# SysCV/LiDAR_snow_sim

Hardware: NVIDIA H100
Metric: augmented LiDAR points/sec (higher is better)
Workload: dtype f64

## Files before the change

### lidar_snow_sim_b200/csrc/api.cu

```cuda
#include "common.cuh"
#include <cmath>
#include <cstring>
#include <cstdlib>

namespace {

void host_range_grid(double *R)
{
    const double stop = 120 + 299792458.0 * 1e-8;
    const double step = stop / (LSS_M_EXT - 1);
    for (int k = 0; k < LSS_M_EXT; k++) {
        double v = (k == LSS_M_EXT - 1) ? stop : k * step;
        R[k] = std::nearbyint(v * 100.0) / 100.0;
    }
}

void host_phase_table(const double *R, double *tab )
{
    const long double ctau = (long double)(299792458.0 * 1e-8);
    const long double pi = 3.14159265358979323846264338327950288L;
    for (int k = 0; k < LSS_M_EXT; k++) {
        const long double a = fmodl((long double)R[k] / ctau, 2.0L);
        tab[2 * k] = (double)sinl(pi * a);
        tab[2 * k + 1] = (double)cosl(pi * a);
    }
}

}

extern "C" {

int lss_version(void) { return 100; }

const char *lss_status_string(lss_status s)
{
    switch (s) {
        case LSS_OK: return "ok";
        case LSS_ERR_INVALID_ARG: return "invalid argument";
        case LSS_ERR_CUDA: return "CUDA error";
        case LSS_ERR_NO_TABLE: return "particle table set not found";
        case LSS_ERR_RANGE_INDEX: return "waveform index out of range (return beyond ~120 m on an occluded beam)";
        case LSS_ERR_NEGATIVE_INTENSITY: return "new intensity is negative";
        case LSS_ERR_OCCLUDER_OVERFLOW: return "too many occluders on one beam";
        case LSS_ERR_WORKSPACE: return "workspace too small";
        case LSS_ERR_NO_SENSOR: return "sensor / camera constants not set";
        case LSS_ERR_TOO_FEW_GROUND: return "fewer than 3 ground points: laser parameters cannot be estimated";
        case LSS_ERR_INTENSITY_RANGE:
            return "intensity histogram range (5, max(I/cos)) of the ground points is not finite or max is below 5";
    }
    return "unknown status";
}

const char *lss_last_error(const lss_engine *e) { return e ? e->last_error.c_str() : "null engine"; }

lss_status lss_create(int device, lss_engine **out)
{
    if (!out) return LSS_ERR_INVALID_ARG;
    *out = nullptr;
    int n_dev = 0;
    if (cudaGetDeviceCount(&n_dev) != cudaSuccess || n_dev == 0) return LSS_ERR_CUDA;
    if (device < 0 || device >= n_dev) return LSS_ERR_INVALID_ARG;
    lss_engine *e = new lss_engine();
    e->device = device;
    DeviceGuard g(device);
    double R[LSS_M_EXT];
    host_range_grid(R);
    std::vector<double> wtab(2 * LSS_M_EXT);
    host_phase_table(R, wtab.data());
    int zero = 0;
    cudaDeviceGetAttribute(&e->n_sm, cudaDevAttrMultiProcessorCount, device);
    if (e->n_sm <= 0) e->n_sm = 132;
    if (cudaMalloc(&e->d_R, sizeof(R)) != cudaSuccess || cudaMalloc(&e->d_status, sizeof(int)) != cudaSuccess ||
        cudaMalloc(&e->d_wtab, sizeof(double) * wtab.size()) != cudaSuccess ||
        cudaMemcpy(e->d_wtab, wtab.data(), sizeof(double) * wtab.size(), cudaMemcpyHostToDevice) != cudaSuccess ||
        cudaMalloc(&e->d_sensor, sizeof(SensorConst)) != cudaSuccess ||
        cudaMalloc(&e->d_camera, sizeof(CameraConst)) != cudaSuccess ||
        cudaMemcpy(e->d_R, R, sizeof(R), cudaMemcpyHostToDevice) != cudaSuccess ||
        cudaMemcpy(e->d_status, &zero, sizeof(int), cudaMemcpyHostToDevice) != cudaSuccess) {
        lss_destroy(e);
        return LSS_ERR_CUDA;
    }
    *out = e;
    return LSS_OK;
}

void lss_destroy(lss_engine *e)
{
    if (!e) return;
    DeviceGuard g(e->device);
    for (auto &kv : e->tables) {
        cudaFree(kv.second.d_rec);
        cudaFree(kv.second.d_tan);
        cudaFree(kv.second.d_plane_off);
        cudaFree(kv.second.d_entries);
        cudaFree(kv.second.d_bucket_start);
    }
    cudaFree(e->d_R);
    cudaFree(e->d_wtab);
    cudaFree(e->d_status);
    cudaFree(e->d_sensor);
    cudaFree(e->d_camera);
    lss_host_pipe_free(e);
    for (cudaStream_t st : e->side) if (st) { cudaStreamSynchronize(st); cudaStreamDestroy(st); }
    for (cudaEvent_t ev : e->side_ev) if (ev) cudaEventDestroy(ev);
    for (auto &sl : e->stage) {
        if (sl.done) { cudaEventSynchronize(sl.done); cudaEventDestroy(sl.done); }
        if (sl.host) cudaFreeHost(sl.host);
    }
    delete e;
}

lss_status lss_set_sensor(lss_engine *e, int n_channels, const double *fd, const double *fs, const double *mi,
                          const double *mx)
{
    if (!e || !fd || !fs || !mi || !mx) return LSS_ERR_INVALID_ARG;
    if (n_channels != LSS_N_CHANNELS) return lss_fail(e, LSS_ERR_INVALID_ARG, "n_channels must be 64");
    DeviceGuard g(e->device);
    for (int c = 0; c < LSS_N_CHANNELS; c++) {
        const double focal_distance = fd[c] * 100;
        const double t = 1 - focal_distance / 13100;
        e->sensor.focal_offset[c] = t * t;
        e->sensor.focal_slope[c] = fs[c];
        e->sensor.min_intensity[c] = mi[c];
        e->sensor.max_intensity[c] = mx[c];
    }
    LSS_CUDA_CHECK(e, cudaMemcpy(e->d_sensor, &e->sensor, sizeof(SensorConst), cudaMemcpyHostToDevice));
    e->has_sensor = true;
    return LSS_OK;
}

lss_status lss_set_camera(lss_engine *e, const float *P2, const float *R0, const float *V2C, int img_h, int img_w)
{
    if (!e || !P2 || !R0 || !V2C) return LSS_ERR_INVALID_ARG;
    DeviceGuard g(e->device);
    for (int k = 0; k < 4; k++)
        for (int j = 0; j < 3; j++) {
            float acc = 0.0f;
            for (int m = 0; m < 3; m++) acc = fmaf(V2C[m * 4 + k], R0[j * 3 + m], acc);
            e->camera.M[k * 3 + j] = acc;
        }
    memcpy(e->camera.P2, P2, sizeof(float) * 12);
    e->camera.img_h = img_h;
    e->camera.img_w = img_w;
    LSS_CUDA_CHECK(e, cudaMemcpy(e->d_camera, &e->camera, sizeof(CameraConst), cudaMemcpyHostToDevice));
    e->has_camera = true;
    return LSS_OK;
}

static lss_status upload_common(lss_engine *e, int n_planes, const double *d_xyr, const int64_t *h_off, double max_div,
                                int n_buckets, cudaStream_t stream, int *id_out)
{
    if (n_planes <= 0 || !h_off || !id_out) return lss_fail(e, LSS_ERR_INVALID_ARG, "bad table arguments");
    if (n_buckets <= 0) n_buckets = 2048;
    if (n_buckets < 8 || n_buckets > (1 << 16)) return lss_fail(e, LSS_ERR_INVALID_ARG, "n_azimuth_buckets out of range");
    if (!(max_div > 0) || max_div > 1.0) return lss_fail(e, LSS_ERR_INVALID_ARG, "max_beam_divergence_rad out of range");
    for (int k = 0; k < n_planes; k++)
        if (h_off[k + 1] < h_off[k] || h_off[0] != 0) return lss_fail(e, LSS_ERR_INVALID_ARG, "bad plane offsets");
    TableSet ts;
    ts.n_planes = n_planes;
    ts.n_buckets = n_buckets;
    ts.max_div_rad = max_div;
    lss_status st = lss_build_tables(e, ts, d_xyr, h_off, stream);
    if (st != LSS_OK) {
        cudaFree(ts.d_rec);
        cudaFree(ts.d_tan);
        cudaFree(ts.d_plane_off);
        cudaFree(ts.d_entries);
        cudaFree(ts.d_bucket_start);
        return st;
    }
    const int id = e->next_table_id++;
    e->tables[id] = ts;
    *id_out = id;
    return LSS_OK;
}

lss_status lss_upload_particles(lss_engine *e, int n_planes, const double *h_xyr, const int64_t *h_off, double max_div,
                                int n_buckets, void *stream, int *id_out)
{
    if (!e || !h_xyr || !h_off) return LSS_ERR_INVALID_ARG;
    DeviceGuard g(e->device);
    cudaStream_t st = (cudaStream_t)stream;
    const int64_t np = n_planes > 0 ? h_off[n_planes] : 0;
    if (np <= 0) return lss_fail(e, LSS_ERR_INVALID_ARG, "empty particle table set");
    double *d_xyr = nullptr;
    LSS_CUDA_CHECK(e, cudaMalloc(&d_xyr, sizeof(double) * 3 * np));
    cudaError_t ce = cudaMemcpyAsync(d_xyr, h_xyr, sizeof(double) * 3 * np, cudaMemcpyHostToDevice, st);
    lss_status r = LSS_OK;
    if (ce != cudaSuccess) {
        e->last_error = cudaGetErrorString(ce);
        r = LSS_ERR_CUDA;
    } else {
        r = upload_common(e, n_planes, d_xyr, h_off, max_div, n_buckets, st, id_out);
    }
    cudaStreamSynchronize(st);
    cudaFree(d_xyr);
    return r;
}

lss_status lss_upload_particles_device(lss_engine *e, int n_planes, const double *d_xyr, const int64_t *h_off,
                                       double max_div, int n_buckets, void *stream, int *id_out)
{
    if (!e || !d_xyr || !h_off) return LSS_ERR_INVALID_ARG;
    DeviceGuard g(e->device);
    return upload_common(e, n_planes, d_xyr, h_off, max_div, n_buckets, (cudaStream_t)stream, id_out);
}

lss_status lss_free_particles(lss_engine *e, int table_id)
{
    if (!e) return LSS_ERR_INVALID_ARG;
    auto it = e->tables.find(table_id);
    if (it == e->tables.end()) return lss_fail(e, LSS_ERR_NO_TABLE, "unknown table id");
    DeviceGuard g(e->device);
    cudaFree(it->second.d_rec);
    cudaFree(it->second.d_tan);
    cudaFree(it->second.d_plane_off);
    cudaFree(it->second.d_entries);
    cudaFree(it->second.d_bucket_start);
    e->tables.erase(it);
    return LSS_OK;
}

lss_status lss_table_info(lss_engine *e, int table_id, int64_t *n_particles, int64_t *n_entries, int64_t *bytes)
{
    if (!e) return LSS_ERR_INVALID_ARG;
    auto it = e->tables.find(table_id);
    if (it == e->tables.end()) return lss_fail(e, LSS_ERR_NO_TABLE, "unknown table id");
    if (n_particles) *n_particles = it->second.n_particles;
    if (n_entries) *n_entries = it->second.n_entries;
    if (bytes) *bytes = it->second.bytes;
    return LSS_OK;
}

int64_t lss_snowfall_workspace_bytes(int64_t n_total, int n_clouds) { return lss_snowfall_ws_bytes(n_total, n_clouds); }

lss_status lss_snowfall_batch(lss_engine *e, int table_id, const float *d_points, const int64_t *h_cloud_offsets,
                              int n_clouds, const int32_t *h_order, double beam_divergence_deg, const float *d_theta,
                              const double *h_thresh_poly, const double *h_plane_in, const int32_t *h_ymins_in,
                              double noise_floor, uint32_t flags, float *d_out_points,
                              int32_t *d_out_counts, double *d_out_stats, float *d_out_full, int32_t *d_out_perm,
                              int32_t *d_out_nocc, void *d_workspace, int64_t workspace_bytes, void *stream)
{
    return lss_snowfall_batch_slots(e, table_id, d_points, h_cloud_offsets, nullptr, n_clouds, h_order,
                                    beam_divergence_deg, d_theta, h_thresh_poly, h_plane_in, h_ymins_in, noise_floor,
                                    flags, d_out_points, d_out_counts, d_out_stats, d_out_full, d_out_perm, d_out_nocc,
                                    d_workspace, workspace_bytes, stream);
}

lss_status lss_snowfall_batch_slots(lss_engine *e, int table_id, const float *d_points, const int64_t *h_cloud_offsets,
                                    const int32_t *d_cloud_counts, int n_clouds, const int32_t *h_order,
                                    double beam_divergence_deg, const float *d_theta, const double *h_thresh_poly,
                                    const double *h_plane_in, const int32_t *h_ymins_in, double noise_floor,
                                    uint32_t flags, float *d_out_points, int32_t *d_out_counts, double *d_out_stats,
                                    float *d_out_full, int32_t *d_out_perm, int32_t *d_out_nocc, void *d_workspace,
                                    int64_t workspace_bytes, void *stream)
{
    if (!e) return LSS_ERR_INVALID_ARG;
    if (!h_cloud_offsets || !h_order || n_clouds < 0 || !d_out_points || !d_out_counts || !d_out_stats)
        return lss_fail(e, LSS_ERR_INVALID_ARG, "null argument");
    if (!d_points && n_clouds <= 65535 && h_cloud_offsets[n_clouds] > 0) return lss_fail(e, LSS_ERR_INVALID_ARG, "null points");
    if (!e->has_sensor) return lss_fail(e, LSS_ERR_NO_SENSOR, "sensor constants not set (lss_set_sensor)");
    auto it = e->tables.find(table_id);
    if (it == e->tables.end()) return lss_fail(e, LSS_ERR_NO_TABLE, "unknown table id");
    DeviceGuard g(e->device);
    SnowfallArgs a;
    a.ts = &it->second;
    a.d_points = d_points;
    a.h_cloud_offsets = h_cloud_offsets;
    a.d_cloud_counts = d_cloud_counts;
    a.n_clouds = n_clouds;
    a.h_order = h_order;
    a.beam_divergence_deg = beam_divergence_deg;
    a.d_theta = d_theta;
    a.h_thresh_poly = h_thresh_poly;
    a.h_plane_in = h_plane_in;
    a.h_ymins_in = h_ymins_in;
    a.noise_floor = noise_floor;
    a.flags = flags;
    a.d_out_points = d_out_points;
    a.d_out_counts = d_out_counts;
    a.d_out_stats = d_out_stats;
    a.d_out_full = d_out_full;
    a.d_out_perm = d_out_perm;
    a.d_out_nocc = d_out_nocc;
    a.d_workspace = d_workspace;
    a.workspace_bytes = workspace_bytes;
    return lss_snowfall_run(e, a, (cudaStream_t)stream);
}

static int64_t *poly_carve(WsCarve &c, void *&pre, int64_t &pre_bytes, int64_t n_total, int n_clouds)
{
    int64_t *off = c.take<int64_t>(n_clouds + 1);
    pre_bytes = lss_prepass_ws_bytes(n_total, n_clouds);
    pre = c.take<char>(pre_bytes);
    return off;
}

int64_t lss_prepass_workspace_bytes(int64_t n_total, int n_clouds)
{
    if (n_total < 0 || n_clouds < 0) return -1;
    WsCarve c;
    void *pre;
    int64_t pre_bytes;
    poly_carve(c, pre, pre_bytes, n_total, n_clouds);
    return c.used;
}

lss_status lss_noise_threshold_poly(lss_engine *e, const float *d_points, const int64_t *h_cloud_offsets, int n_clouds,
                                    double noise_floor, const double *h_plane_in, const int32_t *h_ymins_in,
                                    double *d_poly_out, double *d_plane_out, double *d_fit_out, int32_t *d_ymins_out,
                                    void *d_workspace, int64_t workspace_bytes, void *stream)
{
    if (!e) return LSS_ERR_INVALID_ARG;
    if (!d_points || n_clouds <= 0 || !d_poly_out || !d_workspace) return lss_fail(e, LSS_ERR_INVALID_ARG, "null argument");
    BatchGeometry geo;
    if (lss_status rc = lss_batch_geometry(e, h_cloud_offsets, n_clouds, 0, geo)) return rc;
    DeviceGuard g(e->device);
    if (lss_status rc = lss_prepass_check(e, h_cloud_offsets, n_clouds, h_plane_in != nullptr)) return rc;
    cudaStream_t st = (cudaStream_t)stream;
    WsCarve c{(char *)d_workspace};
    void *d_pre;
    int64_t pre_bytes;
    int64_t *d_off = poly_carve(c, d_pre, pre_bytes, geo.n, n_clouds);
    if (workspace_bytes < c.used) return lss_fail(e, LSS_ERR_WORKSPACE, "workspace too small");
    LSS_CUDA_CHECK(e, lss_stage_upload(e, d_off, h_cloud_offsets, sizeof(int64_t) * (n_clouds + 1), st));
    PrepassIO io;
    io.h_plane_in = h_plane_in;
    io.h_ymins_in = h_ymins_in;
    io.d_poly_out = d_poly_out;
    io.d_plane_out = d_plane_out;
    io.d_fit_out = d_fit_out;
    io.d_ymins_out = d_ymins_out;
    return lss_prepass_run(e, d_points, d_off, nullptr, h_cloud_offsets, n_clouds, 0.5, noise_floor, 0, 0, 1, io,
                           d_pre, pre_bytes, nullptr, st);
}

lss_status lss_check_async(lss_engine *e, void *stream)
{
    if (!e) return LSS_ERR_INVALID_ARG;
    DeviceGuard g(e->device);
    cudaStream_t st = (cudaStream_t)stream;
    int code = 0, zero = 0;
    LSS_CUDA_CHECK(e, cudaStreamSynchronize(st));
    LSS_CUDA_CHECK(e, cudaMemcpyAsync(&code, e->d_status, sizeof(int), cudaMemcpyDeviceToHost, st));
    LSS_CUDA_CHECK(e, cudaStreamSynchronize(st));
    if (code != 0) {
        LSS_CUDA_CHECK(e, cudaMemcpyAsync(e->d_status, &zero, sizeof(int), cudaMemcpyHostToDevice, st));
        LSS_CUDA_CHECK(e, cudaStreamSynchronize(st));
        e->last_error = lss_status_string((lss_status)code);
    }
    return (lss_status)code;
}

int64_t lss_launch_count(const lss_engine *e) { return e ? e->launches : 0; }

lss_status lss_set_profiling(lss_engine *e, int enable)
{
    if (!e) return LSS_ERR_INVALID_ARG;
    e->profiling = enable != 0;
    return LSS_OK;
}

static const char *kernel_names[LSS_K_COUNT] = {"channel_sort", "prepass", "snowfall", "compact", "keep", "wet_ground", "fog",
                                                "snowfall_scan", "snowfall_solve", "voxelize", "dror", "lisa", "fog_lut", "mie",
                                                "select", "pa_aug"};

const char *lss_kernel_name(int kernel) { return (kernel >= 0 && kernel < LSS_K_COUNT) ? kernel_names[kernel] : ""; }

lss_status lss_kernel_times(lss_engine *e, int reset, double *h_ms, int64_t *h_calls, int n)
{
    if (!e || !h_ms || !h_calls) return LSS_ERR_INVALID_ARG;
    DeviceGuard g(e->device);
    for (auto &t : e->timed) {
        float ms = 0.0f;
        if (cudaEventSynchronize(t.end) == cudaSuccess && cudaEventElapsedTime(&ms, t.beg, t.end) == cudaSuccess) {
            e->kernel_ms[t.kernel] += ms;
            e->kernel_calls[t.kernel]++;
        }
        cudaEventDestroy(t.beg);
        cudaEventDestroy(t.end);
    }
    e->timed.clear();
    for (int k = 0; k < n && k < LSS_K_COUNT; k++) { h_ms[k] = e->kernel_ms[k]; h_calls[k] = e->kernel_calls[k]; }
    if (reset) for (int k = 0; k < 16; k++) { e->kernel_ms[k] = 0; e->kernel_calls[k] = 0; }
    return LSS_OK;
}

lss_status lss_debug_range_grid(double *h_out)
{
    if (!h_out) return LSS_ERR_INVALID_ARG;
    host_range_grid(h_out);
    return LSS_OK;
}

}
```

### lidar_snow_sim_b200/csrc/common.cuh

```cuda
#pragma once
#include <cuda_runtime.h>
#include <stdint.h>
#include <stdio.h>
#include <string>
#include <vector>
#include <cstring>
#include <map>
#include <utility>

#include "../../include/lidar_snow_sim.h"

#define LSS_PI 3.141592653589793
#define LSS_TWO_PI 6.283185307179586
#define LSS_M_EXT 1230
#define LSS_ANG_MARGIN 1e-5

struct ParticleRec {
    double phi;
    double rho;
    double alpha;
};
struct ParticleTan {
    double t_right, t_left;
};

typedef uint2 BroadEntry;
#define LSS_RHO_UNIT 0.0025f
#define LSS_RHO_PER_M 400.0
#define LSS_PHI_UNIT 9.587672516830327e-05
#define LSS_IDX_BITS 22
struct EntryView { float x, y, z; int idx; };
__device__ __forceinline__ EntryView lss_decode(const BroadEntry raw, float zbase)
{
    EntryView v;
    v.x = (float)(raw.x & 0xffffu) * LSS_RHO_UNIT;
    v.y = (float)((int)raw.x >> 16) * (float)LSS_PHI_UNIT;
    v.z = zbase * exp2f((float)(raw.y >> LSS_IDX_BITS) * (1.0f / 32.0f));
    v.idx = (int)(raw.y & ((1u << LSS_IDX_BITS) - 1u));
    return v;
}

struct TableSet {
    int n_planes = 0;
    int n_buckets = 0;
    double max_div_rad = 0.0;
    int64_t n_particles = 0;
    int64_t n_entries = 0;
    float zbase = 0.0f;
    ParticleRec *d_rec = nullptr;
    ParticleTan *d_tan = nullptr;
    BroadEntry *d_entries = nullptr;
    int32_t *d_bucket_start = nullptr;
    int64_t *d_plane_off = nullptr;
    int64_t bytes = 0;
};

struct SensorConst {
    double focal_offset[LSS_N_CHANNELS];
    double focal_slope[LSS_N_CHANNELS];
    double min_intensity[LSS_N_CHANNELS];
    double max_intensity[LSS_N_CHANNELS];
};

struct CameraConst {
    float M[12];
    float P2[12];
    int img_h, img_w;
};

__device__ __forceinline__ bool lss_camera_fov(const CameraConst *cam, float out_x, float out_y, float out_z,
                                               const int *img_h, const int *img_w)
{
    const float *M = cam->M, *P2 = cam->P2;
    float rx = fmaf(out_z, M[6], fmaf(out_y, M[3], out_x * M[0])) + M[9];
    float ry = fmaf(out_z, M[7], fmaf(out_y, M[4], out_x * M[1])) + M[10];
    float rz = fmaf(out_z, M[8], fmaf(out_y, M[5], out_x * M[2])) + M[11];
    float u = fmaf(rz, P2[2], fmaf(ry, P2[1], rx * P2[0])) + P2[3];
    float v = fmaf(rz, P2[6], fmaf(ry, P2[5], rx * P2[4])) + P2[7];
    float wd = fmaf(rz, P2[10], fmaf(ry, P2[9], rx * P2[8])) + P2[11];
    u = u / rz;
    v = v / rz;
    const float depth = wd - P2[11];
    return (u >= 0.0f) && (u < (float)*img_w) && (v >= 0.0f) && (v < (float)*img_h) && (depth >= 0.0f);
}

struct lss_host_pipe;
struct lss_engine {
    int device = 0;
    bool has_sensor = false;
    bool has_camera = false;
    SensorConst sensor;
    CameraConst camera;
    SensorConst *d_sensor = nullptr;
    CameraConst *d_camera = nullptr;
    double *d_R = nullptr;
    double2 *d_wtab = nullptr;
    int n_sm = 132;
    int *d_status = nullptr;
    std::map<int, TableSet> tables;
    int next_table_id = 1;
    int64_t launches = 0;
    std::string last_error;
    bool profiling = false;
    struct TimedLaunch { int kernel; cudaEvent_t beg, end; };
    std::vector<TimedLaunch> timed;
    double kernel_ms[16] = {0};
    int64_t kernel_calls[16] = {0};
    struct StageSlot { void *host = nullptr; size_t cap = 0; cudaEvent_t done = nullptr; };
    static constexpr int N_STAGE = 256;
    StageSlot stage[N_STAGE];
    int stage_next = 0;
    static constexpr int N_SIDE = 4;
    cudaStream_t side[N_SIDE] = {};
    cudaEvent_t side_ev[2 * 32] = {};
    int side_next = 0;
    struct lss_host_pipe *pipe = nullptr;
};
void lss_host_pipe_free(lss_engine *e);

inline int64_t align_up(int64_t v, int64_t al) { return (v + al - 1) / al * al; }

struct WsCarve {
    char *base = nullptr;
    int64_t used = 0;
    template <typename T> T *take(int64_t count)
    {
        T *p = base ? (T *)(base + used) : nullptr;
        used = align_up(used + count * (int64_t)sizeof(T), 256);
        return p;
    }
};

template <typename... P, typename... A>
[[nodiscard]] inline cudaError_t lss_launch(lss_engine *e, void (*kernel)(P...), dim3 grid, dim3 block, size_t smem,
                                            cudaStream_t stream, A &&...args)
{
    kernel<<<grid, block, smem, stream>>>(std::forward<A>(args)...);
    e->launches++;
    return cudaGetLastError();
}

inline cudaError_t lss_side_stream(lss_engine *e, cudaStream_t *stream, cudaEvent_t *ev_fork, cudaEvent_t *ev_join)
{
    cudaError_t err;
    const int k = e->side_next++;
    cudaStream_t &s = e->side[k % lss_engine::N_SIDE];
    if (!s) {
        int least = 0, greatest = 0;
        if ((err = cudaDeviceGetStreamPriorityRange(&least, &greatest)) != cudaSuccess) return err;
        if ((err = cudaStreamCreateWithPriority(&s, cudaStreamNonBlocking, greatest)) != cudaSuccess) return err;
    }
    cudaEvent_t *ev = &e->side_ev[2 * (k % 32)];
    for (int j = 0; j < 2; j++)
        if (!ev[j] && (err = cudaEventCreateWithFlags(&ev[j], cudaEventDisableTiming)) != cudaSuccess) return err;
    *stream = s; *ev_fork = ev[0]; *ev_join = ev[1];
    return cudaSuccess;
}

static __global__ void k_stage_copy(uint32_t *dst, const uint32_t *src, int n_words)
{
    for (int i = blockIdx.x * blockDim.x + threadIdx.x; i < n_words; i += gridDim.x * blockDim.x) dst[i] = src[i];
}

inline cudaError_t lss_stage_upload(lss_engine *e, void *dst, const void *src, size_t bytes, cudaStream_t stream)
{
    if (bytes == 0) return cudaSuccess;
    if (bytes % 4 != 0 || ((uintptr_t)dst & 3) != 0) return cudaErrorInvalidValue;
    lss_engine::StageSlot &sl = e->stage[e->stage_next];
    e->stage_next = (e->stage_next + 1) % lss_engine::N_STAGE;
    cudaError_t err;
    if (!sl.done) {
        if ((err = cudaEventCreateWithFlags(&sl.done, cudaEventDisableTiming)) != cudaSuccess) return err;
    } else if ((err = cudaEventSynchronize(sl.done)) != cudaSuccess) {
        return err;
    }
    if (sl.cap < bytes) {
        if (sl.host) cudaFreeHost(sl.host);
        sl.host = nullptr; sl.cap = 0;
        const size_t cap = bytes < 4096 ? 4096 : bytes * 2;
        if ((err = cudaHostAlloc(&sl.host, cap, cudaHostAllocMapped)) != cudaSuccess) return err;
        sl.cap = cap;
    }
    memcpy(sl.host, src, bytes);
    const int n_words = (int)(bytes / 4);
    const int blocks = n_words >= 1 << 16 ? 64 : (n_words + 1023) / 1024;
    if ((err = lss_launch(e, k_stage_copy, blocks, 256, 0, stream, (uint32_t *)dst, (const uint32_t *)sl.host, n_words)) !=
        cudaSuccess)
        return err;
    return cudaEventRecord(sl.done, stream);
}

struct ZeroRegions {
    static constexpr int MAX = 6;
    uint32_t *p[MAX];
    unsigned long long words[MAX];
    int n = 0;
    void add(void *ptr, size_t bytes) { if (ptr && bytes) { p[n] = (uint32_t *)ptr; words[n] = (bytes + 3) / 4; n++; } }
};
static __global__ void k_zero_regions(ZeroRegions r)
{
    uint32_t *p = r.p[blockIdx.y];
    const unsigned long long n = r.words[blockIdx.y];
    const unsigned long long stride = (unsigned long long)gridDim.x * blockDim.x;
    for (unsigned long long i = (unsigned long long)blockIdx.x * blockDim.x + threadIdx.x; i < n; i += stride) p[i] = 0u;
}
inline cudaError_t lss_zero_async(lss_engine *e, const ZeroRegions &r, cudaStream_t stream)
{
    if (r.n == 0) return cudaSuccess;
    unsigned long long mx = 0;
    for (int i = 0; i < r.n; i++) mx = r.words[i] > mx ? r.words[i] : mx;
    const unsigned long long cap = 4ull * e->n_sm;
    const unsigned blocks = (unsigned)((mx + 1023) / 1024 < cap ? (mx + 1023) / 1024 : cap);
    return lss_launch(e, k_zero_regions, dim3(blocks ? blocks : 1, r.n), 256, 0, stream, r);
}

enum { LSS_K_SORT = 0, LSS_K_PREPASS = 1, LSS_K_SNOWFALL = 2, LSS_K_COMPACT = 3, LSS_K_FINALIZE = 4, LSS_K_WET = 5,
       LSS_K_FOG = 6, LSS_K_SCAN = 7, LSS_K_SOLVE = 8, LSS_K_VOXEL = 9, LSS_K_DROR = 10, LSS_K_LISA = 11,
       LSS_K_FOG_LUT = 12, LSS_K_MIE = 13, LSS_K_SELECT = 14, LSS_K_PA = 15, LSS_K_COUNT = 16 };

struct KernelTimer {
    lss_engine *e; cudaStream_t s; int idx = -1;
    KernelTimer(lss_engine *e_, int kernel, cudaStream_t s_) : e(e_), s(s_) {
        if (!e->profiling) return;
        lss_engine::TimedLaunch t; t.kernel = kernel;
        cudaEventCreate(&t.beg); cudaEventCreate(&t.end);
        cudaEventRecord(t.beg, s);
        e->timed.push_back(t); idx = (int)e->timed.size() - 1;
    }
    ~KernelTimer() { if (idx >= 0) cudaEventRecord(e->timed[idx].end, s); }
};

#define LSS_CUDA_CHECK(e, call)                                                                          \
    do {                                                                                                 \
        cudaError_t _err = (call);                                                                       \
        if (_err != cudaSuccess) {                                                                       \
            char _buf[512];                                                                              \
            snprintf(_buf, sizeof(_buf), "%s failed: %s (%s:%d)", #call, cudaGetErrorString(_err),      \
                     __FILE__, __LINE__);                                                                \
            (e)->last_error = _buf;                                                                      \
            return LSS_ERR_CUDA;                                                                         \
        }                                                                                                \
    } while (0)

struct DeviceGuard {
    int prev = -1;
    explicit DeviceGuard(int dev) { cudaGetDevice(&prev); if (prev != dev) cudaSetDevice(dev); else prev = -1; }
    ~DeviceGuard() { if (prev >= 0) cudaSetDevice(prev); }
};

static inline lss_status lss_fail(lss_engine *e, lss_status s, const char *msg)
{
    if (e) e->last_error = msg;
    return s;
}

struct BatchGeometry {
    int64_t n = 0, max_n = 0;
    std::vector<int32_t> tile_base;
};

inline lss_status lss_batch_geometry(lss_engine *e, const int64_t *h_cloud_offsets, int n_clouds, int tile,
                                     BatchGeometry &g)
{
    if (!h_cloud_offsets || n_clouds < 0) return lss_fail(e, LSS_ERR_INVALID_ARG, "null argument");
    if (n_clouds > 65535) return lss_fail(e, LSS_ERR_INVALID_ARG, "at most 65535 clouds per call");
    if (h_cloud_offsets[0] != 0) return lss_fail(e, LSS_ERR_INVALID_ARG, "cloud_offsets[0] must be 0");
    g.max_n = 0;
    g.tile_base.assign(tile > 0 ? n_clouds + 1 : 0, 0);
    for (int b = 0; b < n_clouds; b++) {
        const int64_t n = h_cloud_offsets[b + 1] - h_cloud_offsets[b];
        if (n < 0) return lss_fail(e, LSS_ERR_INVALID_ARG, "cloud_offsets must be non-decreasing");
        if (n >= (1LL << 31)) return lss_fail(e, LSS_ERR_INVALID_ARG, "cloud too large");
        g.max_n = n > g.max_n ? n : g.max_n;
        if (tile > 0) g.tile_base[b + 1] = g.tile_base[b] + (int32_t)((n + tile - 1) / tile);
    }
    g.n = h_cloud_offsets[n_clouds];
    return LSS_OK;
}

inline cudaError_t lss_stage_geometry(lss_engine *e, const int64_t *h_cloud_offsets, int n_clouds,
                                      const std::vector<int32_t> &tile_base, int64_t *d_off, int32_t *d_tile_base,
                                      cudaStream_t stream)
{
    const cudaError_t err = lss_stage_upload(e, d_off, h_cloud_offsets, sizeof(int64_t) * (n_clouds + 1), stream);
    if (err != cudaSuccess) return err;
    return lss_stage_upload(e, d_tile_base, tile_base.data(), sizeof(int32_t) * tile_base.size(), stream);
}

lss_status lss_build_tables(lss_engine *e, TableSet &ts, const double *d_xyr, const int64_t *h_plane_offsets,
                            cudaStream_t stream);
struct SnowfallArgs {
    const TableSet *ts;
    const float *d_points;
    const int64_t *h_cloud_offsets;
    const int32_t *d_cloud_counts = nullptr;
    int n_clouds;
    const int32_t *h_order;
    double beam_divergence_deg;
    const float *d_theta;
    const double *h_thresh_poly;
    const double *h_plane_in = nullptr;
    const int32_t *h_ymins_in = nullptr;
    double noise_floor;
    uint32_t flags;
    float *d_out_points;
    int32_t *d_out_counts;
    double *d_out_stats;
    float *d_out_full;
    int32_t *d_out_perm;
    int32_t *d_out_nocc;
    void *d_workspace;
    int64_t workspace_bytes;
};
lss_status lss_snowfall_run(lss_engine *e, const SnowfallArgs &a, cudaStream_t stream);
struct CloudPre {
    double w[3], h;
    double nw;
    int n_window;
    int n_ground;
    double ymax;
    double lin[2];
    double pmin[2];
    double poly[3];
    float z_med, mad;
    int best_trial;
    int flat;
    double mom[11];
};
__device__ __forceinline__ bool lss_intensity_range_ok(double ymax) { return ymax >= 5.0 && !isinf(ymax); }
__device__ __forceinline__ double lss_plane_dot(double x, double y, double z, const double *w)
{
    return __dadd_rn(__dadd_rn(__dmul_rn(x, w[0]), __dmul_rn(y, w[1])), __dmul_rn(z, w[2]));
}
int64_t lss_prepass_ws_bytes(int64_t n_total, int n_clouds);
struct PrepassIO {
    const double *h_plane_in = nullptr;
    const int32_t *h_ymins_in = nullptr;
    double *d_poly_out = nullptr;
    double *d_plane_out = nullptr;
    double *d_fit_out = nullptr;
    int32_t *d_ymins_out = nullptr;
    int range_min_ground = 3;
};
lss_status lss_prepass_run(lss_engine *e, const float *d_pts, const int64_t *d_cloud_off, const int32_t *d_cloud_cnt,
                           const int64_t *h_cloud_off, int n_clouds, double delta, double noise_floor, int flat_earth,
                           int range64, int raise_few_ground, const PrepassIO &io, void *d_ws, int64_t ws_bytes,
                           void **cloudpre_out, cudaStream_t stream);
lss_status lss_prepass_check(lss_engine *e, const int64_t *h_cloud_off, int n_clouds, bool plane_given);
int64_t lss_snowfall_ws_bytes(int64_t n_total, int n_clouds);
struct DevArgs;
int *lss_snowfall_carve(WsCarve &c, DevArgs &a, void *&prepass, int64_t n_total, int n_clouds);
```

### lidar_snow_sim_b200/csrc/prepass.cu

```cuda
#include "common.cuh"

namespace {

constexpr int PP_TPB = 256;
constexpr int HIST_NX = 50, HIST_NY = 2555;
constexpr int RANSAC_T = 128;


struct PreArgs {
    const float *pts;
    const int64_t *cloud_off;
    const int32_t *cloud_cnt;
    int raise_few;
    int range_min_ground;
    int range64;
    int n_clouds;
    double delta;
    double noise_floor;
    int flat_earth;
    int have_plane;
    CloudPre *cp;
    float *win;
    float *stage;
    int *tile_cnt;
    const int32_t *tile_base;
    double *rec_norm;
    unsigned char *rec_bin;
    int *rec_cnt;
    double *trial;
    double *partial;
    int max_blocks;
    int *status;
    const int32_t *ymins_in;
    int32_t *ymins;
};

__device__ __forceinline__ float range32(float x, float y, float z)
{
    return __fsqrt_rn(__fadd_rn(__fadd_rn(__fmul_rn(x, x), __fmul_rn(y, y)), __fmul_rn(z, z)));
}

__device__ __forceinline__ unsigned long long splitmix64(unsigned long long x)
{
    x += 0x9E3779B97F4A7C15ULL;
    x = (x ^ (x >> 30)) * 0xBF58476D1CE4E5B9ULL;
    x = (x ^ (x >> 27)) * 0x94D049BB133111EBULL;
    return x ^ (x >> 31);
}

template <int NV>
__device__ void block_sum(double (&v)[NV], double *smem )
{
    const int lane = threadIdx.x & 31, warp = threadIdx.x >> 5, nw = blockDim.x >> 5;
#pragma unroll
    for (int k = 0; k < NV; k++)
#pragma unroll
        for (int s = 16; s > 0; s >>= 1) v[k] += __shfl_down_sync(0xffffffffu, v[k], s);
    __syncthreads();
    if (lane == 0)
#pragma unroll
        for (int k = 0; k < NV; k++) smem[k * nw + warp] = v[k];
    __syncthreads();
    if (threadIdx.x == 0)
#pragma unroll
        for (int k = 0; k < NV; k++) {
            double s = 0.0;
            for (int q = 0; q < nw; q++) s += smem[k * nw + q];
            v[k] = s;
        }
}

constexpr int WTILE = 256;

__device__ __forceinline__ bool lss_in_window(float x, float y, float z)
{
    const float lim = __fsub_rn(-1.86f, __fmul_rn(0.01f, x));
    return (z < -1.55f) && (z > lim) && (x > 10.0f) && (x < 70.0f) && (y > -3.0f) && (y < 3.0f);
}
__device__ __forceinline__ int64_t lss_window_tile0(int64_t cloud_begin, int b) { return cloud_begin / 32 + b; }

__global__ void __launch_bounds__(WTILE) k_window_tiles(PreArgs a)
{
    const int b = blockIdx.y;
    const int64_t beg = a.cloud_off[b];
    const int n = (a.cloud_cnt ? a.cloud_cnt[b] : (int)(a.cloud_off[b + 1] - beg));
    const int w0 = blockIdx.x * WTILE + (threadIdx.x & ~31);
    if (w0 >= n) return;
    const int lane = threadIdx.x & 31;
    const int i = w0 + lane;
    float x = 0, y = 0, z = 0;
    bool in = false;
    if (i < n) {
        const float *r = a.pts + (beg + i) * 5;
        x = __ldcs(r); y = __ldcs(r + 1); z = __ldcs(r + 2);
        in = lss_in_window(x, y, z);
    }
    const unsigned m = __ballot_sync(0xffffffffu, in);
    if (in) {
        float *o = a.stage + (beg + w0 + __popc(m & ((1u << lane) - 1u))) * 3;
        o[0] = x; o[1] = y; o[2] = z;
    }
    if (lane == 0) a.tile_cnt[lss_window_tile0(beg, b) + w0 / 32] = __popc(m);
}

__device__ __forceinline__ unsigned f2key(float f)
{
    unsigned u = __float_as_uint(f);
    return (u & 0x80000000u) ? ~u : (u | 0x80000000u);
}
__device__ __forceinline__ float key2f(unsigned k)
{
    unsigned u = (k & 0x80000000u) ? (k & 0x7fffffffu) : ~k;
    return __uint_as_float(u);
}

__device__ float block_select(const float *win, int K, int kth, int mode, float centre, unsigned *hist ,
                              unsigned *bcast )
{
    unsigned prefix = 0, mask = 0;
    int k = kth;
    for (int shift = 24; shift >= 0; shift -= 8) {
        for (int q = threadIdx.x; q < 256; q += blockDim.x) hist[q] = 0;
        __syncthreads();
        for (int i = threadIdx.x; i < K; i += blockDim.x) {
            float v = win[3 * (size_t)i + 2];
            if (mode) v = fabsf(__fsub_rn(v, centre));
            const unsigned key = f2key(v);
            if ((key & mask) == prefix) atomicAdd(&hist[(key >> shift) & 255u], 1u);
        }
        __syncthreads();
        if (threadIdx.x == 0) {
            int acc = 0;
            unsigned d = 0;
            for (; d < 256; d++) {
                if (acc + (int)hist[d] > k) break;
                acc += (int)hist[d];
            }
            bcast[0] = d;
            bcast[1] = (unsigned)(k - acc);
        }
        __syncthreads();
        prefix |= bcast[0] << shift;
        mask |= 255u << shift;
        k = (int)bcast[1];
        __syncthreads();
    }
    return key2f(prefix);
}

__device__ float block_median(const float *win, int K, int mode, float centre, unsigned *hist, unsigned *bcast)
{
    const float hi = block_select(win, K, K / 2, mode, centre, hist, bcast);
    if (K & 1) return hi;
    const float lo = block_select(win, K, K / 2 - 1, mode, centre, hist, bcast);
    return __fmul_rn(__fadd_rn(lo, hi), 0.5f);
}

__global__ void __launch_bounds__(1024) k_window_gather_mad(PreArgs a)
{
    extern __shared__ int prefix[];
    __shared__ int wsum[32];
    __shared__ int run_s;
    __shared__ unsigned hist[256];
    __shared__ unsigned bcast[2];
    const int b = blockIdx.x;
    const int64_t beg = a.cloud_off[b];
    const int n = (a.cloud_cnt ? a.cloud_cnt[b] : (int)(a.cloud_off[b + 1] - beg));
    const int n_tiles = (n + 31) / 32;
    const int *cnt = a.tile_cnt + lss_window_tile0(beg, b);
    const int tid = threadIdx.x, lane = tid & 31, warp = tid >> 5;
    if (tid == 0) run_s = 0;
    __syncthreads();
    for (int base = 0; base < n_tiles; base += 1024) {
        const int t = base + tid;
        const int v = t < n_tiles ? cnt[t] : 0;
        int incl = v;
#pragma unroll
        for (int s = 1; s < 32; s <<= 1) { const int o = __shfl_up_sync(0xffffffffu, incl, s); if (lane >= s) incl += o; }
        if (lane == 31) wsum[warp] = incl;
        __syncthreads();
        int o = run_s;
        for (int wv = 0; wv < warp; wv++) o += wsum[wv];
        if (t < n_tiles) prefix[t] = o + incl - v;
        __syncthreads();
        if (tid == 1023) run_s = o + incl;
        __syncthreads();
    }
    if (tid == 0) { prefix[n_tiles] = run_s; a.cp[b].n_window = run_s; }
    __syncthreads();
    const int K = prefix[n_tiles];
    float *win = a.win + beg * 3;
    for (int o = tid; o < K; o += blockDim.x) {
        int lo = 0, hi = n_tiles;
        while (hi - lo > 1) { const int mid = (lo + hi) >> 1; if (prefix[mid] <= o) lo = mid; else hi = mid; }
        const float *src = a.stage + (beg + (int64_t)lo * 32 + (o - prefix[lo])) * 3;
        float *dst = win + (int64_t)o * 3;
        dst[0] = src[0]; dst[1] = src[1]; dst[2] = src[2];
    }
    if (K <= 5) return;
    __syncthreads();
    const float med = block_median(win, K, 0, 0.0f, hist, bcast);
    const float mad = block_median(win, K, 1, med, hist, bcast);
    if (threadIdx.x == 0) { a.cp[b].z_med = med; a.cp[b].mad = mad; }
}

__global__ void __launch_bounds__(PP_TPB) k_ransac_trials(PreArgs a)
{
    __shared__ double red[5 * (PP_TPB / 32)];
    __shared__ double model[4];
    const int b = blockIdx.y, t = blockIdx.x;
    const int K = a.cp[b].n_window;
    double *out = a.trial + ((size_t)b * RANSAC_T + t) * 8;
    if (K <= 5) { if (threadIdx.x == 0) out[5] = 0.0; return; }
    const float *win = a.win + a.cloud_off[b] * 3;
    if (threadIdx.x == 0) {
        unsigned long long s = splitmix64(0x5851F42D4C957F2DULL ^ ((unsigned long long)(unsigned)K << 32) ^ (unsigned)t);
        int i0 = (int)(s % (unsigned)K);
        s = splitmix64(s);
        int i1 = (int)(s % (unsigned)(K - 1));
        if (i1 >= i0) i1++;
        s = splitmix64(s);
        int i2 = (int)(s % (unsigned)(K - 2));
        const int lo = i0 < i1 ? i0 : i1, hi = i0 < i1 ? i1 : i0;
        if (i2 >= lo) i2++;
        if (i2 >= hi) i2++;
        const double x0 = win[3 * i0], y0 = win[3 * i0 + 1], z0 = win[3 * i0 + 2];
        const double x1 = win[3 * i1] - x0, y1 = win[3 * i1 + 1] - y0, z1 = win[3 * i1 + 2] - z0;
        const double x2 = win[3 * i2] - x0, y2 = win[3 * i2 + 1] - y0, z2 = win[3 * i2 + 2] - z0;
        const double det = x1 * y2 - x2 * y1;
        double valid = 0.0, pa = 0, pb = 0, pc = 0;
        if (fabs(det) > 1e-9) {
            pa = (z1 * y2 - z2 * y1) / det;
            pb = (x1 * z2 - x2 * z1) / det;
            pc = z0 - pa * x0 - pb * y0;
            valid = 1.0;
        }
        model[0] = pa; model[1] = pb; model[2] = pc; model[3] = valid;
    }
    __syncthreads();
    if (model[3] == 0.0) { if (threadIdx.x == 0) out[5] = 0.0; return; }
    const double pa = model[0], pb = model[1], pc = model[2];
    const double thr = (double)a.cp[b].mad;
    double v[5] = {0, 0, 0, 0, 0};
    for (int i = threadIdx.x; i < K; i += PP_TPB) {
        const double x = win[3 * i], y = win[3 * i + 1], z = win[3 * i + 2];
        const double r = z - (pa * x + pb * y + pc);
        const double r2 = r * r;
        if (r2 <= thr) { v[0] += 1.0; v[1] += r2; v[2] += z; v[3] += z * z; }
    }
    block_sum<5>(v, red);
    if (threadIdx.x == 0) {
        const double n = v[0];
        const double ss_tot = v[3] - (n > 0 ? v[2] * v[2] / n : 0.0);
        out[0] = n;
        out[1] = (n > 0 && ss_tot > 0) ? 1.0 - v[1] / ss_tot : -1e300;
        out[2] = pa; out[3] = pb; out[4] = pc;
        out[5] = n >= 3 ? 1.0 : 0.0;
    }
}

__global__ void __launch_bounds__(PP_TPB) k_ransac_refit(PreArgs a)
{
    __shared__ double red[6 * (PP_TPB / 32)];
    __shared__ double bc[8];
    const int b = blockIdx.x;
    CloudPre &cp = a.cp[b];
    const int K = cp.n_window;
    if (threadIdx.x < 32) {
        int best = -1;
        double bn = -1, bs = -1e301;
        for (int t = threadIdx.x; t < RANSAC_T && K > 5; t += 32) {
            const double *tr = a.trial + ((size_t)b * RANSAC_T + t) * 8;
            if (tr[5] == 0.0) continue;
            if (tr[0] > bn || (tr[0] == bn && tr[1] > bs)) { bn = tr[0]; bs = tr[1]; best = t; }
        }
#pragma unroll
        for (int sft = 16; sft > 0; sft >>= 1) {
            const double on = __shfl_xor_sync(0xffffffffu, bn, sft), os = __shfl_xor_sync(0xffffffffu, bs, sft);
            const int ob = __shfl_xor_sync(0xffffffffu, best, sft);
            const bool take = ob >= 0 && (best < 0 || on > bn || (on == bn && (os > bs || (os == bs && ob < best))));
            if (take) { bn = on; bs = os; best = ob; }
        }
        if (threadIdx.x == 0) {
        cp.best_trial = best;
        bc[0] = (double)best;
        if (best >= 0) {
            const double *tr = a.trial + ((size_t)b * RANSAC_T + best) * 8;
            bc[1] = tr[2]; bc[2] = tr[3]; bc[3] = tr[4];
        }
        }
    }
    __syncthreads();
    const int best = (int)bc[0];
    if (best < 0) {
        if (threadIdx.x == 0) { cp.w[0] = 0; cp.w[1] = 0; cp.w[2] = 1; cp.h = -1.55; cp.nw = 1.0; cp.flat = 1; }
        return;
    }
    const float *win = a.win + a.cloud_off[b] * 3;
    const double pa = bc[1], pb = bc[2], pc = bc[3], thr = (double)cp.mad;
    double m[6] = {0, 0, 0, 0, 0, 0};
    for (int i = threadIdx.x; i < K; i += PP_TPB) {
        const double x = win[3 * i], y = win[3 * i + 1], z = win[3 * i + 2];
        const double r = z - (pa * x + pb * y + pc);
        if (r * r <= thr) { m[0] += 1.0; m[1] += x; m[2] += y; m[3] += z; }
    }
    block_sum<6>(m, red);
    if (threadIdx.x == 0) { bc[4] = m[0]; bc[5] = m[1] / m[0]; bc[6] = m[2] / m[0]; bc[7] = m[3] / m[0]; }
    __syncthreads();
    const double xm = bc[5], ym = bc[6], zm = bc[7];
    double c[6] = {0, 0, 0, 0, 0, 0};
    for (int i = threadIdx.x; i < K; i += PP_TPB) {
        const double x = win[3 * i], y = win[3 * i + 1], z = win[3 * i + 2];
        const double r = z - (pa * x + pb * y + pc);
        if (r * r <= thr) {
            const double dx = x - xm, dy = y - ym, dz = z - zm;
            c[0] += dx * dx; c[1] += dx * dy; c[2] += dy * dy; c[3] += dx * dz; c[4] += dy * dz;
        }
    }
    block_sum<6>(c, red);
    if (threadIdx.x == 0) {
        const double det = c[0] * c[2] - c[1] * c[1];
        double fa = pa, fb = pb, fc = pc;
        if (fabs(det) > 1e-12 * (c[0] * c[2] + 1e-300)) {
            fa = (c[3] * c[2] - c[4] * c[1]) / det;
            fb = (c[0] * c[4] - c[1] * c[3]) / det;
            fc = zm - fa * xm - fb * ym;
        }
        const double nrm = sqrt(fa * fa + fb * fb + 1.0);
        cp.w[0] = fa / nrm; cp.w[1] = fb / nrm; cp.w[2] = -1.0 / nrm; cp.h = fc;
        cp.nw = sqrt(cp.w[0] * cp.w[0] + cp.w[1] * cp.w[1] + cp.w[2] * cp.w[2]);
        cp.flat = 0;
    }
}

__global__ void k_set_plane(PreArgs a, const double *plane )
{
    const int b = blockIdx.x * blockDim.x + threadIdx.x;
    if (b >= a.n_clouds) return;
    CloudPre &cp = a.cp[b];
    cp.w[0] = plane[4 * b]; cp.w[1] = plane[4 * b + 1]; cp.w[2] = plane[4 * b + 2]; cp.h = plane[4 * b + 3];
    cp.nw = sqrt(cp.w[0] * cp.w[0] + cp.w[1] * cp.w[1] + cp.w[2] * cp.w[2]);
    cp.flat = 0;
    cp.best_trial = -2;
}

struct GroundPt { bool ground; double d, cosang, norm_i; };

__device__ __forceinline__ GroundPt ground_point(const PreArgs &a, const CloudPre &cp, const float *r)
{
    GroundPt g;
    const double x = r[0], y = r[1], z = r[2];
    const double pw = lss_plane_dot(x, y, z, cp.w);
    const double hgt = pw + cp.h;
    g.ground = (hgt < a.delta) && (hgt > -a.delta);
    if (!g.ground) { g.d = 0.0; g.cosang = 0.0; g.norm_i = 0.0; return g; }
    g.d = a.range64 ? sqrt((x * x + y * y) + z * z) : (double)range32(r[0], r[1], r[2]);
    double c;
    if (a.flat_earth) c = -(z) / (g.d * 1.0);
    else c = pw / (g.d * cp.nw);
    g.cosang = (c >= -1.0 && c <= 1.0) ? c : __longlong_as_double(0x7ff8000000000000LL);
    g.norm_i = (double)r[3] / g.cosang;
    return g;
}

__device__ __forceinline__ int edge_bin(double v, double lo, double hi, int nb)
{
    if (!(v >= lo) || !(v <= hi)) return -1;
    const double step = (hi - lo) / nb;
    int k = (int)((v - lo) / step);
    k = k < 0 ? 0 : (k > nb ? nb : k);
    while (k > 0 && v < ((k == nb) ? hi : (k * step + lo))) k--;
    while (k < nb && v >= ((k + 1 == nb) ? hi : ((k + 1) * step + lo))) k++;
    if (k >= nb) k = nb - 1;
    return k;
}

__device__ __forceinline__ void intensity_edges(double ymax, double &lo, double &hi)
{
    lo = ymax == 5.0 ? 4.5 : 5.0;
    hi = ymax == 5.0 ? 5.5 : ymax;
}

__device__ __forceinline__ double nan_max(double a, double b) { return (a != a || a > b) ? a : b; }

__device__ __forceinline__ int ground_blocks(int n, int launched)
{
    return min(launched, max(1, (n + PP_TPB * 8 - 1) / (PP_TPB * 8)));
}

__global__ void __launch_bounds__(PP_TPB) k_ground_stats(PreArgs a)
{
    __shared__ double red[15 * (PP_TPB / 32)];
    __shared__ double mx[PP_TPB / 32];
    const int b = blockIdx.y;
    const CloudPre cp = a.cp[b];
    const int64_t beg = a.cloud_off[b];
    const int n = (a.cloud_cnt ? a.cloud_cnt[b] : (int)(a.cloud_off[b + 1] - beg));
    const int nb = ground_blocks(n, gridDim.x);
    if ((int)blockIdx.x >= nb) return;
    const int lane = threadIdx.x & 31;
    double v[15] = {0, 0, 0, 0, 0, 0, 0, 0, 0, 0, 0, 0, 0, 0, 0};
    double vmax = -1e300;
    for (int w0 = blockIdx.x * PP_TPB + (threadIdx.x & ~31); w0 < n; w0 += nb * PP_TPB) {
        const int i = w0 + lane;
        GroundPt g;
        g.ground = false;
        if (i < n) {
            const float *r = a.pts + (beg + i) * 5;
            const float row[4] = {__ldcs(r), __ldcs(r + 1), __ldcs(r + 2), __ldcs(r + 3)};
            g = ground_point(a, cp, row);
        }
        int bx = -1;
        if (g.ground) {
            const double dd = g.d - 30.0, yy = g.norm_i - 50.0;
            v[0] += 1.0; v[1] += dd; v[2] += yy; v[3] += dd * dd; v[4] += dd * yy;
            vmax = nan_max(vmax, g.norm_i);
            const double t = (g.d - 40.0) / 30.0, t2 = t * t;
            const double c = g.cosang, dc = g.d * g.cosang;
            v[5] += t; v[6] += t2; v[7] += t2 * t; v[8] += t2 * t2;
            v[9] += c; v[10] += c * t; v[11] += c * t2;
            v[12] += dc; v[13] += dc * t; v[14] += dc * t2;
            if (g.norm_i >= 4.5) bx = edge_bin(g.d, 10.0, 70.0, HIST_NX);
        }
        const unsigned m = __ballot_sync(0xffffffffu, bx >= 0);
        if (m) {
            int k0 = 0;
            if (lane == 0) k0 = atomicAdd(&a.rec_cnt[b], __popc(m));
            k0 = __shfl_sync(0xffffffffu, k0, 0);
            if (bx >= 0) {
                const int64_t k = beg + k0 + __popc(m & ((1u << lane) - 1u));
                a.rec_norm[k] = g.norm_i;
                a.rec_bin[k] = (unsigned char)bx;
            }
        }
    }
#pragma unroll
    for (int s = 16; s > 0; s >>= 1) vmax = nan_max(vmax, __shfl_down_sync(0xffffffffu, vmax, s));
    if ((threadIdx.x & 31) == 0) mx[threadIdx.x >> 5] = vmax;
    block_sum<15>(v, red);
    if (threadIdx.x == 0) {
        for (int q = 0; q < PP_TPB / 32; q++) vmax = nan_max(vmax, mx[q]);
        double *p = a.partial + ((size_t)b * a.max_blocks + blockIdx.x) * 16;
        for (int k = 0; k < 15; k++) p[k] = v[k];
        p[15] = vmax;
    }
}

template <int NV>
__device__ __forceinline__ void warp_reduce_partials(const double *partial, int n_blocks, double (&v)[NV], double *vmax)
{
    const int lane = threadIdx.x & 31;
#pragma unroll
    for (int k = 0; k < NV; k++) v[k] = 0.0;
    double m = -1e300;
    for (int q = lane; q < n_blocks; q += 32) {
        const double *p = partial + (size_t)q * 16;
#pragma unroll
        for (int k = 0; k < NV; k++) v[k] += p[k];
        if (vmax) m = nan_max(m, p[NV]);
    }
#pragma unroll
    for (int s = 16; s > 0; s >>= 1) {
#pragma unroll
        for (int k = 0; k < NV; k++) v[k] += __shfl_xor_sync(0xffffffffu, v[k], s);
        m = nan_max(m, __shfl_xor_sync(0xffffffffu, m, s));
    }
    if (vmax) *vmax = m;
}

#ifndef LSS_HIST_SLAB
#define LSS_HIST_SLAB 5
#endif
constexpr int HIST_SLAB = LSS_HIST_SLAB, HIST_SLABS = (HIST_NX + HIST_SLAB - 1) / HIST_SLAB, HIST_TPB = 512;

__global__ void __launch_bounds__(HIST_TPB) k_ground_hist(PreArgs a, int n_blocks)
{
    extern __shared__ unsigned hist[];
    __shared__ double stat[2];
    const int b = blockIdx.y, bx0 = blockIdx.x * HIST_SLAB;
    const int nbx = min(HIST_SLAB, HIST_NX - bx0);
    const int lane = threadIdx.x & 31, warp = threadIdx.x >> 5;
    if (warp == 0) {
        double v[15], vmax;
        const int n = a.cloud_cnt ? a.cloud_cnt[b] : (int)(a.cloud_off[b + 1] - a.cloud_off[b]);
        warp_reduce_partials<15>(a.partial + (size_t)b * a.max_blocks * 16, ground_blocks(n, n_blocks), v, &vmax);
        if (lane == 0) {
            stat[0] = v[0];
            stat[1] = fabs(vmax);
            if (blockIdx.x == 0) {
                CloudPre &cp = a.cp[b];
                cp.n_ground = (int)v[0];
                cp.mom[0] = v[0];
                for (int k = 0; k < 10; k++) cp.mom[1 + k] = v[5 + k];
                cp.ymax = fabs(vmax);
                if (v[0] >= 3.0) {
                    const double n = v[0], mx_ = v[1] / n, my_ = v[2] / n;
                    const double sxx = v[3] - n * mx_ * mx_, sxy = v[4] - n * mx_ * my_;
                    const double slope = sxy / sxx;
                    cp.lin[0] = slope;
                    cp.lin[1] = (my_ + 50.0) - slope * (mx_ + 30.0);
                } else {
                    cp.lin[0] = cp.lin[1] = 0.0;
                    if (a.raise_few) atomicMax(a.status, LSS_ERR_TOO_FEW_GROUND);
                }
                if (v[0] >= (double)a.range_min_ground && !lss_intensity_range_ok(cp.ymax))
                    atomicMax(a.status, LSS_ERR_INTENSITY_RANGE);
            }
        }
    }
    __syncthreads();
    const int n_ground = (int)stat[0];
    const double ymax = stat[1];
    if (n_ground < 3 || !lss_intensity_range_ok(ymax)) return;
    double ylo, yhi;
    intensity_edges(ymax, ylo, yhi);
    int32_t *ymins = a.ymins + b * HIST_NX + bx0;
    if (a.ymins_in) {
        for (int k = threadIdx.x; k < nbx; k += HIST_TPB) {
            const int inj = a.ymins_in[b * HIST_NX + bx0 + k];
            ymins[k] = inj < 0 ? 0 : (inj >= HIST_NY ? HIST_NY - 1 : inj);
        }
        return;
    }
    for (int k = threadIdx.x; k < nbx * HIST_NY; k += HIST_TPB) hist[k] = 0;
    __syncthreads();
    const int64_t beg = a.cloud_off[b];
    const int n_rec = a.rec_cnt[b];
    const unsigned char *bins = a.rec_bin + beg;
    const double *norms = a.rec_norm + beg;
    constexpr int U = 4;
    for (int k0 = threadIdx.x; k0 < n_rec; k0 += U * HIST_TPB) {
        int rel[U];
#pragma unroll
        for (int u = 0; u < U; u++) {
            const int k = k0 + u * HIST_TPB;
            rel[u] = k < n_rec ? (int)bins[k] - bx0 : -1;
        }
#pragma unroll
        for (int u = 0; u < U; u++)
            if ((unsigned)rel[u] < (unsigned)nbx) {
                const int by = edge_bin(norms[k0 + u * HIST_TPB], ylo, yhi, HIST_NY);
                if (by >= 0) atomicAdd(&hist[rel[u] * HIST_NY + by], 1u);
            }
    }
    __syncthreads();
    for (int w = warp; w < nbx; w += HIST_TPB / 32) {
        unsigned best = 0xffffffffu;
        int bidx = 0x7fffffff;
        for (int k = lane; k < HIST_NY; k += 32) {
            unsigned c = hist[w * HIST_NY + k];
            if (c == 0) c = (unsigned)n_ground;
            if (c < best) { best = c; bidx = k; }
        }
        for (int s = 16; s > 0; s >>= 1) {
            const unsigned ob = __shfl_down_sync(0xffffffffu, best, s);
            const int oi = __shfl_down_sync(0xffffffffu, bidx, s);
            if (ob < best || (ob == best && oi < bidx)) { best = ob; bidx = oi; }
        }
        if (lane == 0) ymins[w] = bidx;
    }
}

__device__ __forceinline__ bool minima_point(int k, int bidx, double ylo, double yhi, double ystep, double &x, double &y)
{
    y = (bidx == HIST_NY) ? yhi : __dadd_rn(__dmul_rn((double)bidx, ystep), ylo);
    const double e0 = k * (60.0 / HIST_NX) + 10.0;
    const double e1 = (k + 1 == HIST_NX) ? 70.0 : ((k + 1) * (60.0 / HIST_NX) + 10.0);
    x = (e0 + e1) / 2;
    return y > 5.0;
}

__global__ void k_poly_solve(PreArgs a, double *poly_out , double *plane_out ,
                             double *fit_out , int32_t *ymins_out )
{
    const int b = blockIdx.x;
    CloudPre &cp = a.cp[b];
    if (threadIdx.x != 0) return;
    const bool picked = cp.n_ground >= 3 && lss_intensity_range_ok(cp.ymax);
    if (cp.n_ground >= 3) {
        const int32_t *ymins = a.ymins + b * HIST_NX;
        double ylo, yhi;
        intensity_edges(cp.ymax, ylo, yhi);
        const double ystep = (yhi - ylo) / HIST_NY;
        int m = 0;
        double sx = 0, sy = 0, x, y;
        for (int k = 0; k < HIST_NX && picked; k++)
            if (minima_point(k, ymins[k], ylo, yhi, ystep, x, y)) { m++; sx += x; sy += y; }
        if (m > 3) {
            const double mx_ = sx / m, my_ = sy / m;
            double sxx = 0, sxy = 0;
            for (int k = 0; k < HIST_NX; k++)
                if (minima_point(k, ymins[k], ylo, yhi, ystep, x, y)) { sxx += (x - mx_) * (x - mx_); sxy += (x - mx_) * (y - my_); }
            cp.pmin[0] = sxy / sxx;
            cp.pmin[1] = my_ - cp.pmin[0] * mx_;
        } else {
            cp.pmin[0] = cp.lin[0];
            cp.pmin[1] = cp.lin[1];
        }
    }
    double s[8];
    s[0] = cp.mom[0]; s[1] = cp.mom[1]; s[2] = cp.mom[2]; s[3] = cp.mom[3]; s[4] = cp.mom[4];
    for (int k = 0; k < 3; k++) s[5 + k] = a.noise_floor * (cp.pmin[0] * cp.mom[8 + k] + cp.pmin[1] * cp.mom[5 + k]);
    double A[3][4] = {{s[0], s[1], s[2], s[5]}, {s[1], s[2], s[3], s[6]}, {s[2], s[3], s[4], s[7]}};
    bool ok = cp.n_ground >= 3;
    for (int c = 0; c < 3 && ok; c++) {
        int piv = c;
        for (int r = c + 1; r < 3; r++) if (fabs(A[r][c]) > fabs(A[piv][c])) piv = r;
        if (fabs(A[piv][c]) < 1e-300) { ok = false; break; }
        for (int k = 0; k < 4; k++) { double t = A[c][k]; A[c][k] = A[piv][k]; A[piv][k] = t; }
        for (int r = c + 1; r < 3; r++) {
            const double f = A[r][c] / A[c][c];
            for (int k = c; k < 4; k++) A[r][k] -= f * A[c][k];
        }
    }
    double c2 = 0, c1 = 0, c0 = 0;
    if (ok) {
        c2 = A[2][3] / A[2][2];
        c1 = (A[1][3] - A[1][2] * c2) / A[1][1];
        c0 = (A[0][3] - A[0][1] * c1 - A[0][2] * c2) / A[0][0];
    }
    const double m = 40.0, sc = 30.0;
    cp.poly[0] = c2 / (sc * sc);
    cp.poly[1] = c1 / sc - 2.0 * c2 * m / (sc * sc);
    cp.poly[2] = c0 - c1 * m / sc + c2 * m * m / (sc * sc);
    if (poly_out) { poly_out[3 * b] = cp.poly[0]; poly_out[3 * b + 1] = cp.poly[1]; poly_out[3 * b + 2] = cp.poly[2]; }
    if (plane_out) { plane_out[4 * b] = cp.w[0]; plane_out[4 * b + 1] = cp.w[1]; plane_out[4 * b + 2] = cp.w[2]; plane_out[4 * b + 3] = cp.h; }
    if (fit_out) {
        double *f = fit_out + 8 * b;
        f[0] = cp.lin[0]; f[1] = cp.lin[1]; f[2] = cp.pmin[0]; f[3] = cp.pmin[1]; f[4] = cp.ymax;
        f[5] = (double)cp.n_ground; f[6] = (double)cp.n_window; f[7] = (double)cp.flat;
    }
    if (ymins_out) for (int k = 0; k < HIST_NX; k++) ymins_out[b * HIST_NX + k] = picked ? a.ymins[b * HIST_NX + k] : -1;
}

}

static void prepass_carve(WsCarve &c, PreArgs &a, double *&plane_in, int32_t *&ymins_in, int64_t n_total, int n_clouds)
{
    a.max_blocks = 64;
    a.cp = c.take<CloudPre>(n_clouds);
    a.rec_cnt = c.take<int>(n_clouds);
    a.win = c.take<float>(n_total * 3);
    a.stage = c.take<float>(n_total * 3);
    a.rec_norm = (double *)a.stage;
    a.rec_bin = a.stage ? (unsigned char *)a.stage + n_total * 8 : nullptr;
    a.tile_cnt = c.take<int>(n_total / 32 + n_clouds + 2);
    a.tile_base = c.take<int32_t>(n_clouds + 1);
    a.trial = c.take<double>((int64_t)n_clouds * RANSAC_T * 8);
    a.partial = c.take<double>((int64_t)n_clouds * a.max_blocks * 16);
    plane_in = c.take<double>((int64_t)n_clouds * 4);
    a.ymins = c.take<int32_t>((int64_t)n_clouds * HIST_NX);
    ymins_in = c.take<int32_t>((int64_t)n_clouds * HIST_NX);
}

int64_t lss_prepass_ws_bytes(int64_t n_total, int n_clouds)
{
    WsCarve c;
    PreArgs a;
    double *plane_in;
    int32_t *ymins_in;
    prepass_carve(c, a, plane_in, ymins_in, n_total, n_clouds);
    return c.used;
}

static size_t gather_dyn_smem(int64_t max_n) { return sizeof(int) * ((size_t)(max_n + 31) / 32 + 2); }

static int64_t largest_cloud(const int64_t *h_cloud_off, int n_clouds)
{
    int64_t max_n = 0;
    for (int b = 0; b < n_clouds; b++) max_n = std::max<int64_t>(max_n, h_cloud_off[b + 1] - h_cloud_off[b]);
    return max_n;
}

static lss_status gather_smem_limits(lss_engine *e, size_t &static_bytes, size_t &optin_bytes)
{
    cudaFuncAttributes fa;
    int optin = 0;
    LSS_CUDA_CHECK(e, cudaFuncGetAttributes(&fa, k_window_gather_mad));
    LSS_CUDA_CHECK(e, cudaDeviceGetAttribute(&optin, cudaDevAttrMaxSharedMemoryPerBlockOptin, e->device));
    static_bytes = fa.sharedSizeBytes;
    optin_bytes = (size_t)optin;
    return LSS_OK;
}

lss_status lss_prepass_check(lss_engine *e, const int64_t *h_cloud_off, int n_clouds, bool plane_given)
{
    if (plane_given || n_clouds <= 0) return LSS_OK;
    const int64_t max_n = largest_cloud(h_cloud_off, n_clouds);
    size_t static_bytes = 0, optin_bytes = 0;
    if (lss_status rc = gather_smem_limits(e, static_bytes, optin_bytes)) return rc;
    if (static_bytes + gather_dyn_smem(max_n) <= optin_bytes) return LSS_OK;
    const int64_t limit = ((int64_t)((optin_bytes - static_bytes) / sizeof(int)) - 2) * 32;
    char msg[256];
    snprintf(msg, sizeof(msg), "pre-pass: a cloud of %lld rows is larger than the %lld rows whose mounting window this "
             "device can gather (shared memory); give its plane or split it", (long long)max_n, (long long)limit);
    e->last_error = msg;
    return LSS_ERR_INVALID_ARG;
}

lss_status lss_prepass_run(lss_engine *e, const float *d_pts, const int64_t *d_cloud_off, const int32_t *d_cloud_cnt,
                           const int64_t *h_cloud_off, int n_clouds, double delta, double noise_floor, int flat_earth,
                           int range64, int raise_few_ground, const PrepassIO &io, void *d_ws, int64_t ws_bytes,
                           void **cloudpre_out, cudaStream_t stream)
{
    const double *h_plane_in = io.h_plane_in;
    double *d_poly_out = io.d_poly_out, *d_plane_out = io.d_plane_out;
    const int B = n_clouds;
    const int64_t N = h_cloud_off[B];
    PreArgs a;
    WsCarve c{(char *)d_ws};
    double *d_plane;
    int32_t *d_ymins_in;
    prepass_carve(c, a, d_plane, d_ymins_in, N, B);
    if (lss_status rc = lss_prepass_check(e, h_cloud_off, B, h_plane_in != nullptr)) return rc;
    if (ws_bytes < c.used) return lss_fail(e, LSS_ERR_WORKSPACE, "pre-pass workspace too small");
    a.pts = d_pts;
    a.cloud_off = d_cloud_off;
    a.cloud_cnt = d_cloud_cnt;
    a.range64 = range64;
    a.raise_few = raise_few_ground;
    a.range_min_ground = io.range_min_ground;
    a.n_clouds = B;
    a.delta = delta;
    a.noise_floor = noise_floor;
    a.flat_earth = flat_earth;
    a.have_plane = h_plane_in != nullptr;
    a.status = e->d_status;
    a.ymins_in = nullptr;
    if (io.h_ymins_in) {
        LSS_CUDA_CHECK(e, lss_stage_upload(e, d_ymins_in, io.h_ymins_in, sizeof(int32_t) * HIST_NX * B, stream));
        a.ymins_in = d_ymins_in;
    }
    if (cloudpre_out) *cloudpre_out = a.cp;
    const int64_t max_n = largest_cloud(h_cloud_off, B);
    int nblk = (int)std::min<int64_t>(a.max_blocks, std::max<int64_t>(1, (max_n + PP_TPB * 8 - 1) / (PP_TPB * 8)));

    {
        ZeroRegions z;
        z.add(a.cp, (size_t)((char *)a.rec_cnt - (char *)a.cp) + sizeof(int) * B);
        LSS_CUDA_CHECK(e, lss_zero_async(e, z, stream));
    }
    {
        KernelTimer kt(e, LSS_K_PREPASS, stream);
        if (h_plane_in) {
            LSS_CUDA_CHECK(e, lss_stage_upload(e, d_plane, h_plane_in, sizeof(double) * 4 * B, stream));
            LSS_CUDA_CHECK(e, lss_launch(e, k_set_plane, (B + 127) / 128, 128, 0, stream, a, d_plane));
        } else {
            const int max_tiles = (int)std::max<int64_t>(1, (max_n + WTILE - 1) / WTILE);
            LSS_CUDA_CHECK(e, lss_launch(e, k_window_tiles, dim3(max_tiles, B), WTILE, 0, stream, a));
            const size_t gather_smem = gather_dyn_smem(max_n);
            size_t static_bytes = 0, optin_bytes = 0;
            if (lss_status rc = gather_smem_limits(e, static_bytes, optin_bytes)) return rc;
            if (static_bytes + gather_smem > 48 * 1024)
                LSS_CUDA_CHECK(e, cudaFuncSetAttribute(k_window_gather_mad, cudaFuncAttributeMaxDynamicSharedMemorySize,
                                                       (int)gather_smem));
            LSS_CUDA_CHECK(e, lss_launch(e, k_window_gather_mad, B, 1024, gather_smem, stream, a));
            LSS_CUDA_CHECK(e, lss_launch(e, k_ransac_trials, dim3(RANSAC_T, B), PP_TPB, 0, stream, a));
            LSS_CUDA_CHECK(e, lss_launch(e, k_ransac_refit, B, PP_TPB, 0, stream, a));
        }
        LSS_CUDA_CHECK(e, lss_launch(e, k_ground_stats, dim3(nblk, B), PP_TPB, 0, stream, a));
        const size_t hist_smem = sizeof(unsigned) * HIST_SLAB * HIST_NY;
        if (hist_smem > 48 * 1024)
            LSS_CUDA_CHECK(e, cudaFuncSetAttribute(k_ground_hist, cudaFuncAttributeMaxDynamicSharedMemorySize, (int)hist_smem));
        LSS_CUDA_CHECK(e, lss_launch(e, k_ground_hist, dim3(HIST_SLABS, B), HIST_TPB, hist_smem, stream, a, nblk));
        LSS_CUDA_CHECK(e, lss_launch(e, k_poly_solve, B, 32, 0, stream, a, d_poly_out, d_plane_out, io.d_fit_out,
                                     io.d_ymins_out));
    }
    return LSS_OK;
}
```

### lidar_snow_sim_b200/csrc/segments.cuh

```cuda
#pragma once
#include "common.cuh"

constexpr int SEG_MAX_K = 2;
constexpr int SEG_SCAN_TPB = 1024;

struct SegTiles {
    const int32_t *tile_base;
    int *tile;
    int32_t *total[SEG_MAX_K];
};

inline SegTiles seg_take(WsCarve &c, int64_t n_total, int n_clouds, int tile, int K)
{
    int32_t *p = c.take<int32_t>((int64_t)(n_clouds + 1) + (n_total / tile + n_clouds + 1) * K);
    SegTiles s{};
    s.tile_base = p;
    s.tile = p ? p + (n_clouds + 1) : nullptr;
    return s;
}

__device__ __forceinline__ int seg_rows(const int64_t *cloud_off, const int32_t *cloud_cnt, int b)
{
    return cloud_cnt ? cloud_cnt[b] : (int)(cloud_off[b + 1] - cloud_off[b]);
}

template <int K>
__device__ __forceinline__ void seg_count(int cls, const SegTiles &s, int b, int tile)
{
    __shared__ int cnt[K];
    if (threadIdx.x < K) cnt[threadIdx.x] = 0;
    __syncthreads();
#pragma unroll
    for (int k = 0; k < K; k++) {
        const unsigned m = __ballot_sync(0xffffffffu, cls == k);
        if ((threadIdx.x & 31) == 0 && m) atomicAdd(&cnt[k], __popc(m));
    }
    __syncthreads();
    if (threadIdx.x < K) s.tile[(size_t)(s.tile_base[b] + tile) * K + threadIdx.x] = cnt[threadIdx.x];
}

template <int K, int TILE>
__device__ __forceinline__ int seg_rank(int cls, const SegTiles &s, int b, int tile)
{
    __shared__ __align__(16) int warp_cnt[K][TILE / 32];
    const int lane = threadIdx.x & 31, warp = threadIdx.x >> 5;
    unsigned mine = 0;
#pragma unroll
    for (int k = 0; k < K; k++) {
        const unsigned m = __ballot_sync(0xffffffffu, cls == k);
        if (lane == 0) warp_cnt[k][warp] = __popc(m);
        if (cls == k) mine = m;
    }
    __syncthreads();
    if (cls < 0) return -1;
    int r = __popc(mine & ((1u << lane) - 1u));
#pragma unroll
    for (int k = 0; k < K; k++) {
        if (cls != k) continue;
        r += s.tile[(size_t)(s.tile_base[b] + tile) * K + k];
        for (int w = 0; w < warp; w++) r += warp_cnt[k][w];
    }
    return r;
}

template <int K, int TILE>
__global__ void __launch_bounds__(TILE) k_seg_count_codes(const uint8_t *code, const int64_t *cloud_off,
                                                          const int32_t *cloud_cnt, SegTiles s)
{
    const int b = blockIdx.y, tile = blockIdx.x;
    if (tile >= s.tile_base[b + 1] - s.tile_base[b]) return;
    const int i = tile * TILE + threadIdx.x;
    int cls = -1;
    if (i < seg_rows(cloud_off, cloud_cnt, b)) {
        const int c = code[cloud_off[b] + i];
        if (c < K) cls = c;
    }
    seg_count<K>(cls, s, b, tile);
}

template <int K>
__global__ void __launch_bounds__(SEG_SCAN_TPB) k_seg_scan(SegTiles s)
{
    __shared__ __align__(16) int warp_sum[K][SEG_SCAN_TPB / 32];
    __shared__ int run[K];
    const int b = blockIdx.x;
    const int t0 = s.tile_base[b], nt = s.tile_base[b + 1] - t0;
    const int lane = threadIdx.x & 31, warp = threadIdx.x >> 5;
    if (threadIdx.x < K) run[threadIdx.x] = 0;
    __syncthreads();
    for (int base = 0; base < nt; base += SEG_SCAN_TPB) {
        const int t = base + threadIdx.x;
        int *c = s.tile + (size_t)(t0 + t) * K;
        int v[K], incl[K], off[K];
#pragma unroll
        for (int k = 0; k < K; k++) {
            v[k] = t < nt ? c[k] : 0;
            incl[k] = v[k];
#pragma unroll
            for (int d = 1; d < 32; d <<= 1) {
                const int u = __shfl_up_sync(0xffffffffu, incl[k], d);
                if (lane >= d) incl[k] += u;
            }
            if (lane == 31) warp_sum[k][warp] = incl[k];
        }
        __syncthreads();
#pragma unroll
        for (int k = 0; k < K; k++) {
            off[k] = run[k];
            for (int w = 0; w < warp; w++) off[k] += warp_sum[k][w];
            if (t < nt) c[k] = off[k] + incl[k] - v[k];
        }
        __syncthreads();
        if (threadIdx.x == SEG_SCAN_TPB - 1) {
#pragma unroll
            for (int k = 0; k < K; k++) run[k] = off[k] + incl[k];
        }
        __syncthreads();
    }
    if (threadIdx.x == 0) {
#pragma unroll
        for (int k = 0; k < K; k++)
            if (s.total[k]) s.total[k][b] = run[k];
    }
}
```

### lidar_snow_sim_b200/csrc/snowfall.cu

```cuda
#include "beam.cuh"

namespace {

constexpr int SCHED_KEY_TPB = 128;

__global__ void __launch_bounds__(SCHED_KEY_TPB) k_sched_key(const float *__restrict__ pts, const int64_t *__restrict__ cloud_off,
                                                            const int32_t *__restrict__ cloud_cnt,
                                                            const int32_t *__restrict__ order, const int32_t *__restrict__ wtile_base,
                                                            unsigned long long *ent, int *hist)
{
    const int b = blockIdx.y, t = blockIdx.x * SCHED_KEY_TPB + threadIdx.x;
    const int64_t beg = cloud_off[b];
    const int n_slot = (int)(cloud_off[b + 1] - beg);
    if (blockIdx.x * SCHED_KEY_TPB * 32 >= n_slot) return;
    const int w0 = 32 * t;
    const bool on = w0 < n_slot;
    int bin = -1;
    if (on) {
        const int ch = w0 < seg_rows(cloud_off, cloud_cnt, b) ? channel_bin(pts[(beg + w0) * 5 + 4]) : LSS_N_CHANNELS;
        bin = ch < LSS_N_CHANNELS ? order[b * LSS_N_CHANNELS + ch] % SCHED_PLANES : SCHED_PLANES;
        ent[wtile_base[b] + t] = ((unsigned long long)bin << 48) | ((unsigned long long)b << 32) | (unsigned)w0;
    }
    const unsigned m = __match_any_sync(0xffffffffu, bin);
    if (on && (threadIdx.x & 31) == __ffs(m) - 1) atomicAdd(&hist[bin], __popc(m));
}

constexpr int HIT_SLOTS_PER_BEAM = 3;
constexpr int SCHED_PER_THREAD = 2;
__global__ void __launch_bounds__(256) k_sched_sort(const unsigned long long *__restrict__ in, unsigned long long *out,
                                                    int *hist, int n)
{
    __shared__ int base[SCHED_BINS], cnt[SCHED_BINS], blk[SCHED_BINS];
    const int first = blockIdx.x * (256 * SCHED_PER_THREAD);
    for (int c = threadIdx.x; c < SCHED_BINS; c += 256) cnt[c] = 0;
    if (threadIdx.x < 32) {
        int run = 0;
        for (int c0 = 0; c0 < SCHED_BINS; c0 += 32) {
            const int c = c0 + (int)threadIdx.x;
            const int v = c < SCHED_BINS ? hist[c] : 0;
            int incl = v;
#pragma unroll
            for (int s = 1; s < 32; s <<= 1) {
                const int t = __shfl_up_sync(0xffffffffu, incl, s);
                if ((int)threadIdx.x >= s) incl += t;
            }
            if (c < SCHED_BINS) base[c] = run + incl - v;
            run += __shfl_sync(0xffffffffu, incl, 31);
        }
    }
    __syncthreads();
    const int lane = threadIdx.x & 31;
    int bin_of[SCHED_PER_THREAD], rank[SCHED_PER_THREAD];
    unsigned long long e[SCHED_PER_THREAD];
#pragma unroll
    for (int k = 0; k < SCHED_PER_THREAD; k++) {
        const int s = first + k * 256 + threadIdx.x;
        const bool on = s < n;
        e[k] = on ? in[s] : 0ull;
        const int bin = on ? (int)(e[k] >> 48) : -1;
        bin_of[k] = bin;
        const unsigned m = __match_any_sync(0xffffffffu, bin);
        const int leader = __ffs(m) - 1;
        int r = 0;
        if (on && lane == leader) r = atomicAdd(&cnt[bin], __popc(m));
        r = __shfl_sync(0xffffffffu, r, leader);
        rank[k] = r + __popc(m & ((1u << lane) - 1u));
    }
    __syncthreads();
    for (int c = threadIdx.x; c < SCHED_BINS; c += 256)
        blk[c] = cnt[c] ? atomicAdd(&hist[SCHED_BINS + c], cnt[c]) : 0;
    __syncthreads();
#pragma unroll
    for (int k = 0; k < SCHED_PER_THREAD; k++)
        if (bin_of[k] >= 0) out[base[bin_of[k]] + blk[bin_of[k]] + rank[k]] = e[k];
}

constexpr int KEEP_TPB = 256;
constexpr int KEEP_ROWS = TILE / KEEP_TPB;

__global__ void __launch_bounds__(KEEP_TPB) k_keep(DevArgs a)
{
    __shared__ unsigned h_keep[NBINS], h_all[NBINS];
    __shared__ int s_cnt[2];
    const int b = blockIdx.y, tile = blockIdx.x;
    const int64_t beg = a.cloud_off[b];
    if (tile * TILE >= (int)(a.cloud_off[b + 1] - beg)) return;
    const int n_tile = seg_rows(a.cloud_off, a.cloud_cnt, b) - tile * TILE;
    if (threadIdx.x < NBINS) { h_keep[threadIdx.x] = 0; h_all[threadIdx.x] = 0; }
    if (threadIdx.x < 2) s_cnt[threadIdx.x] = 0;
    const bool thr_on = a.flags & LSS_FLAG_THRESHOLD_FILTER;
    int tags[KEEP_ROWS];
    float d32s[KEEP_ROWS], out_is[KEEP_ROWS];
#pragma unroll
    for (int k = 0; k < KEEP_ROWS; k++) {
        const int i = tile * TILE + k * KEEP_TPB + threadIdx.x;
        tags[k] = 0; d32s[k] = 0.0f; out_is[k] = 0.0f;
        if (k * KEEP_TPB + (int)threadIdx.x < n_tile) {
            tags[k] = __ldcs(a.keep_tag + beg + i);
            if (thr_on) { d32s[k] = __ldcs(a.keep_d + beg + i); out_is[k] = __ldcs(a.keep_i + beg + i); }
        }
    }
    double p0 = 0.0, p1 = 0.0, p2 = 0.0;
    if (thr_on) { p0 = a.thresh[3 * b]; p1 = a.thresh[3 * b + 1]; p2 = a.thresh[3 * b + 2]; }
    __syncthreads();
    const int lane = threadIdx.x & 31;
#pragma unroll
    for (int k = 0; k < KEEP_ROWS; k++) {
        const int i = tile * TILE + k * KEEP_TPB + threadIdx.x;
        const bool active = k * KEEP_TPB + (int)threadIdx.x < n_tile;
        bool keep = false, att = false;
        int ch = -1;
        if (active) {
            const int label = keep_tag_label(tags[k]);
            ch = tags[k] - NBINS * label;
            keep = true;
            if (thr_on) {
                const float d32 = d32s[k];
                const double d = (double)d32;
                const double d2 = (double)__fmul_rn(d32, d32);
                const double thr = __dadd_rn(__dadd_rn(__dmul_rn(p0, d2), __dmul_rn(p1, d)), p2);
                keep = (label == 2) || ((double)out_is[k] > thr);
            }
            att = keep && label == 1 && ch < LSS_N_CHANNELS;
            if (keep && (a.flags & LSS_FLAG_CAMERA_FOV)) {
                const float *row = a.aug + (beg + i) * 5;
                keep = lss_camera_fov(a.camera, row[0], row[1], row[2], &a.camera->img_h, &a.camera->img_w);
            }
            a.code_keep[beg + i] = keep ? (uint8_t)ch : (uint8_t)255;
            if (a.code_all) a.code_all[beg + i] = (uint8_t)ch;
        }
        const int ck = (active && keep) ? ch : -1;
        const unsigned mk = __match_any_sync(0xffffffffu, ck);
        if (ck >= 0 && lane == __ffs(mk) - 1) atomicAdd(&h_keep[ck], (unsigned)__popc(mk));
        if (a.hist_all) {
            const unsigned ma = __match_any_sync(0xffffffffu, active ? ch : -1);
            if (active && lane == __ffs(ma) - 1) atomicAdd(&h_all[ch], (unsigned)__popc(ma));
        }
        const unsigned m_att = __ballot_sync(0xffffffffu, att);
        const unsigned m_rem = __ballot_sync(0xffffffffu, active && !keep);
        if (lane == 0) {
            if (m_att) atomicAdd(&s_cnt[0], __popc(m_att));
            if (m_rem) atomicAdd(&s_cnt[1], __popc(m_rem));
        }
    }
    __syncthreads();
    if (threadIdx.x < NBINS) {
        const size_t hrow = ((size_t)a.tile_base[b] + tile) * NBINS + threadIdx.x;
        a.hist_keep[hrow] = h_keep[threadIdx.x];
        if (a.hist_all) a.hist_all[hrow] = h_all[threadIdx.x];
    }
    if (threadIdx.x < 2 && s_cnt[threadIdx.x]) atomicAdd(&a.counters[2 * b + threadIdx.x], s_cnt[threadIdx.x]);
}

constexpr int TSCAN_PER_LANE = 4;
constexpr int TSCAN_ADD = 8;

__global__ void __launch_bounds__(1024) k_tile_scan(unsigned *hist, const int32_t *__restrict__ tile_base,
                                                     int32_t *counts , double *stats, const int *counters,
                                                     const unsigned *att_cnt, const unsigned long long *att_sum,
                                                     const SensorConst *sensor)
{
    __shared__ unsigned bin_total[NBINS];
    __shared__ double att_term[LSS_N_CHANNELS];
    const int b = blockIdx.x;
    const int n_tiles = tile_base[b + 1] - tile_base[b];
    unsigned *h = hist + (size_t)tile_base[b] * NBINS;
    const int lane = threadIdx.x & 31, warp = threadIdx.x >> 5;
    if (stats && threadIdx.x < LSS_N_CHANNELS)
        att_term[threadIdx.x] = (double)att_cnt[b * LSS_N_CHANNELS + threadIdx.x] * (0.9 * sensor->max_intensity[threadIdx.x]);
    for (int c = warp; c < NBINS; c += 32) {
        unsigned run = 0;
        for (int t0 = 0; t0 < n_tiles; t0 += 32 * TSCAN_PER_LANE) {
            const int t = t0 + lane * TSCAN_PER_LANE;
            unsigned v[TSCAN_PER_LANE], sum = 0;
#pragma unroll
            for (int q = 0; q < TSCAN_PER_LANE; q++) {
                v[q] = t + q < n_tiles ? h[(size_t)(t + q) * NBINS + c] : 0u;
                sum += v[q];
            }
            unsigned incl = sum;
#pragma unroll
            for (int s = 1; s < 32; s <<= 1) { const unsigned o = __shfl_up_sync(0xffffffffu, incl, s); if (lane >= s) incl += o; }
            unsigned ex = run + incl - sum;
#pragma unroll
            for (int q = 0; q < TSCAN_PER_LANE; q++) {
                if (t + q < n_tiles) h[(size_t)(t + q) * NBINS + c] = ex;
                ex += v[q];
            }
            run += __shfl_sync(0xffffffffu, incl, 31);
        }
        if (lane == 0) bin_total[c] = run;
    }
    __syncthreads();
    if (threadIdx.x == 0) {
        unsigned run = 0;
        for (int c = 0; c < NBINS; c++) { const unsigned t = bin_total[c]; bin_total[c] = run; run += t; }
        if (counts) counts[b] = (int32_t)run;
        if (stats) {
            const int n_att = counters[2 * b], n_rem = counters[2 * b + 1];
            double sum = 0.0;
            for (int c = 0; c < LSS_N_CHANNELS; c++) sum += att_term[c];
            sum -= (double)att_sum[b];
            stats[4 * b + 3] = sum;
            stats[4 * b + 0] = (double)n_att;
            stats[4 * b + 1] = (double)n_rem;
            stats[4 * b + 2] = n_att > 0 ? (double)(long long)(sum / (double)n_att) : 0.0;
        }
    }
    __syncthreads();
    const int total = n_tiles * NBINS;
    for (int k0 = threadIdx.x; k0 < total; k0 += TSCAN_ADD * blockDim.x) {
        unsigned v[TSCAN_ADD];
#pragma unroll
        for (int q = 0; q < TSCAN_ADD; q++) {
            const int k = k0 + q * blockDim.x;
            v[q] = k < total ? h[k] : 0u;
        }
#pragma unroll
        for (int q = 0; q < TSCAN_ADD; q++) {
            const int k = k0 + q * blockDim.x;
            if (k < total) h[k] = v[q] + bin_total[k % NBINS];
        }
    }
}

__global__ void __launch_bounds__(TILE) k_scatter(const float *__restrict__ aug, const uint8_t *__restrict__ code,
                                                   const unsigned *__restrict__ tile_off,
                                                   const int64_t *__restrict__ cloud_off,
                                                   const int32_t *__restrict__ cloud_cnt,
                                                   const int32_t *__restrict__ tile_base,
                                                   float *__restrict__ out, const int32_t *__restrict__ nocc_in,
                                                   int32_t *__restrict__ nocc_out, int32_t *__restrict__ perm_out)
{
    __shared__ unsigned warp_cnt[TILE / 32][NBINS];
    const int b = blockIdx.y, tile = blockIdx.x;
    const int64_t beg = cloud_off[b];
    const int n = seg_rows(cloud_off, cloud_cnt, b);
    const int i = tile * TILE + threadIdx.x;
    if (tile * TILE >= n) return;
    const int lane = threadIdx.x & 31, warp = threadIdx.x >> 5;
    for (int k = threadIdx.x; k < (TILE / 32) * NBINS; k += TILE) (&warp_cnt[0][0])[k] = 0;
    __syncthreads();
    int c = -1;
    if (i < n) {
        const int cc = code[beg + i];
        c = cc < NBINS ? cc : -1;
    }
    const unsigned m = __match_any_sync(0xffffffffu, c);
    const int rank = __popc(m & ((1u << lane) - 1u));
    if (c >= 0 && rank == 0) warp_cnt[warp][c] = __popc(m);
    __syncthreads();
    if (threadIdx.x < NBINS) {
        unsigned run = tile_off[((size_t)tile_base[b] + tile) * NBINS + threadIdx.x];
        for (int wv = 0; wv < TILE / 32; wv++) { const unsigned t = warp_cnt[wv][threadIdx.x]; warp_cnt[wv][threadIdx.x] = run; run += t; }
    }
    __syncthreads();
    if (c >= 0) {
        const int64_t dst = beg + warp_cnt[warp][c] + rank;
        const float *s = aug + (beg + i) * 5;
        float *o = out + dst * 5;
#pragma unroll
        for (int q = 0; q < 5; q++) o[q] = s[q];
        if (nocc_out) nocc_out[dst] = nocc_in[beg + i];
        if (perm_out) perm_out[dst] = i;
    }
}

int64_t hit_cap(int64_t n_total) { return std::min<int64_t>(n_total * HIT_SLOTS_PER_BEAM + 4096, 0x7fffffff); }

int64_t sched_tiles(int64_t n_total, int n_clouds) { return n_total / 32 + (int64_t)n_clouds + 1; }

int64_t att_cnt_off(int n_clouds) { return align_up((int64_t)n_clouds * 2 * 4, 8); }
int64_t counters_bytes(int n_clouds) { return att_cnt_off(n_clouds) + (int64_t)n_clouds * (LSS_N_CHANNELS * 4 + 8); }

}

int *lss_snowfall_carve(WsCarve &c, DevArgs &a, void *&prepass, int64_t n_total, int n_clouds)
{
    const int64_t hist_rows = n_total / TILE + (int64_t)n_clouds + 1;
    a.aug = c.take<float>(n_total * 5);
    a.keep_d = c.take<float>(n_total);
    a.keep_i = c.take<float>(n_total);
    a.keep_tag = c.take<uint8_t>(n_total);
    a.code_keep = c.take<uint8_t>(n_total);
    a.code_all = c.take<uint8_t>(n_total);
    a.nocc = c.take<int32_t>(n_total);
    a.hist_keep = c.take<unsigned>(hist_rows * NBINS);
    a.hist_all = c.take<unsigned>(hist_rows * NBINS);
    a.cloud_off = c.take<int64_t>(n_clouds + 1);
    a.tile_base = c.take<int32_t>((int64_t)(n_clouds + 1) * 2);
    a.order = c.take<int32_t>((int64_t)n_clouds * LSS_N_CHANNELS);
    a.thresh = c.take<double>((int64_t)n_clouds * 3);
    a.counters = (int *)c.take<char>(counters_bytes(n_clouds));
    a.chunks_per_class = (int)((n_total + LIST_CHUNK - 1) / LIST_CHUNK);
    a.hit_cap = (int)hit_cap(n_total);
    a.hdr = (int *)c.take<char>(LIST_HDR_BYTES + (a.chunks_per_class + LIST_CLASSES) * LIST_CHUNK * (int64_t)sizeof(SolveItem) +
                                (int64_t)a.hit_cap * 3 * 8);
    a.chunk_tab = c.take<int>((int64_t)LIST_CLASSES * a.chunks_per_class);
    int *sched = (int *)c.take<char>((int64_t)SCHED_BINS * 2 * 4 + 2 * sched_tiles(n_total, n_clouds) * 8);
    prepass = c.take<char>(lss_prepass_ws_bytes(n_total, n_clouds));
    return sched;
}

int64_t lss_snowfall_ws_bytes(int64_t n_total, int n_clouds)
{
    if (n_total < 0 || n_clouds < 0) return -1;
    WsCarve c;
    DevArgs a;
    void *prepass;
    lss_snowfall_carve(c, a, prepass, n_total, n_clouds);
    return c.used;
}

lss_status lss_snowfall_run(lss_engine *e, const SnowfallArgs &s, cudaStream_t stream)
{
    const int B = s.n_clouds;
    BatchGeometry g, wg;
    if (lss_status rc = lss_batch_geometry(e, s.h_cloud_offsets, B, TILE, g)) return rc;
    if (lss_status rc = lss_batch_geometry(e, s.h_cloud_offsets, B, 32, wg)) return rc;
    const int64_t N = g.n, max_n = g.max_n;
    for (int k = 0; k < B * LSS_N_CHANNELS; k++)
        if (s.h_order[k] < 0 || s.h_order[k] >= s.ts->n_planes)
            return lss_fail(e, LSS_ERR_NO_TABLE, "order[] names a plane that is not in the table set");
    DevArgs a;
    WsCarve c{(char *)s.d_workspace};
    void *d_prepass_ws;
    int *d_sched_hist = lss_snowfall_carve(c, a, d_prepass_ws, N, B);
    if (s.workspace_bytes < c.used || !s.d_workspace) return lss_fail(e, LSS_ERR_WORKSPACE, "workspace too small");
    if ((s.flags & LSS_FLAG_THRESHOLD_FILTER) && !s.h_thresh_poly && !(s.flags & LSS_FLAG_DEVICE_PREPASS))
        return lss_fail(e, LSS_ERR_INVALID_ARG, "threshold filter needs h_thresh_poly or LSS_FLAG_DEVICE_PREPASS");
    if ((s.flags & LSS_FLAG_CAMERA_FOV) && !e->has_camera)
        return lss_fail(e, LSS_ERR_NO_SENSOR, "camera calibration not set");
    const double div_rad = s.beam_divergence_deg * (LSS_PI / 180.0);
    if (!(div_rad > 0) || div_rad > s.ts->max_div_rad * (1 + 1e-12))
        return lss_fail(e, LSS_ERR_INVALID_ARG, "beam_divergence exceeds the value the table set was built for");
    const int max_tiles = (int)((max_n + TILE - 1) / TILE);
    const int n_wtiles = wg.tile_base[B];
    if ((s.d_out_perm || s.d_out_nocc) && !s.d_out_full)
        return lss_fail(e, LSS_ERR_INVALID_ARG, "d_out_perm / d_out_nocc need d_out_full");
    const bool device_prepass = (s.flags & LSS_FLAG_THRESHOLD_FILTER) && (s.flags & LSS_FLAG_DEVICE_PREPASS) &&
                                !s.h_thresh_poly;
    if (device_prepass)
        if (lss_status rc = lss_prepass_check(e, s.h_cloud_offsets, B, s.h_plane_in != nullptr)) return rc;

    const bool want_all = s.d_out_full != nullptr;
    if (!want_all) a.code_all = nullptr, a.hist_all = nullptr;
    if (!s.d_out_nocc) a.nocc = nullptr;
    int64_t *d_off = (int64_t *)a.cloud_off;
    int32_t *d_tile_base = (int32_t *)a.tile_base;
    int32_t *d_order = (int32_t *)a.order;
    double *d_thresh = (double *)a.thresh;
    unsigned *d_att_cnt = (unsigned *)((char *)a.counters + att_cnt_off(B));
    unsigned long long *d_att_sum = (unsigned long long *)((char *)d_att_cnt + (int64_t)B * LSS_N_CHANNELS * 4);

    g.tile_base.insert(g.tile_base.end(), wg.tile_base.begin(), wg.tile_base.end());
    LSS_CUDA_CHECK(e, lss_stage_geometry(e, s.h_cloud_offsets, B, g.tile_base, d_off, d_tile_base, stream));
    LSS_CUDA_CHECK(e, lss_stage_upload(e, d_order, s.h_order, sizeof(int32_t) * B * LSS_N_CHANNELS, stream));
    if (s.h_thresh_poly)
        LSS_CUDA_CHECK(e, lss_stage_upload(e, d_thresh, s.h_thresh_poly, sizeof(double) * 3 * B, stream));
    {
        ZeroRegions z;
        z.add(a.counters, counters_bytes(B));
        z.add(s.d_out_stats, sizeof(double) * 4 * B);
        if (N == 0 || B == 0) {
            z.add(s.d_out_counts, sizeof(int32_t) * B);
            LSS_CUDA_CHECK(e, lss_zero_async(e, z, stream));
            return LSS_OK;
        }
        z.add(a.hdr, LIST_HDR_BYTES);
        z.add(a.chunk_tab, (size_t)LIST_CLASSES * a.chunks_per_class * 4);
        z.add(d_sched_hist, (size_t)SCHED_BINS * 2 * 4);
        LSS_CUDA_CHECK(e, lss_zero_async(e, z, stream));
    }

    a.rec = s.ts->d_rec;
    a.tan = s.ts->d_tan;
    a.plane_off = s.ts->d_plane_off;
    a.zbase = s.ts->zbase;
    a.entries = s.ts->d_entries;
    a.bucket_start = s.ts->d_bucket_start;
    a.n_buckets = s.ts->n_buckets;
    a.n_planes = s.ts->n_planes;
    a.w = LSS_TWO_PI / s.ts->n_buckets;
    a.inv_w = s.ts->n_buckets / LSS_TWO_PI;
    a.pts = s.d_points;
    a.theta = s.d_theta;
    a.cloud_cnt = s.d_cloud_counts;
    a.sensor = e->d_sensor;
    a.camera = e->d_camera;
    a.R = e->d_R;
    a.wtab = e->d_wtab;
    a.half_div = (s.beam_divergence_deg / 2) * (LSS_PI / 180.0);
    a.div_rad = div_rad;
    a.flags = s.flags;
    a.stats = s.d_out_stats;
    a.att_cnt = d_att_cnt;
    a.att_sum = d_att_sum;
    a.status = e->d_status;
    SolveItem *d_solve_list = (SolveItem *)((char *)a.hdr + LIST_HDR_BYTES);
    a.hit_a1 = (double *)(d_solve_list + (a.chunks_per_class + LIST_CLASSES) * LIST_CHUNK);
    a.hit_a2 = a.hit_a1 + a.hit_cap;
    a.hit_rho = a.hit_a2 + a.hit_cap;
    cudaEvent_t ev_join = nullptr;
    if (device_prepass) {
        cudaStream_t side = nullptr;
        cudaEvent_t ev_fork = nullptr;
        LSS_CUDA_CHECK(e, lss_side_stream(e, &side, &ev_fork, &ev_join));
        LSS_CUDA_CHECK(e, cudaEventRecord(ev_fork, stream));
        LSS_CUDA_CHECK(e, cudaStreamWaitEvent(side, ev_fork, 0));
        PrepassIO io;
        io.h_plane_in = s.h_plane_in;
        io.h_ymins_in = s.h_ymins_in;
        io.d_poly_out = d_thresh;
        lss_status ps = lss_prepass_run(e, s.d_points, d_off, s.d_cloud_counts, s.h_cloud_offsets, B, 0.5, s.noise_floor, 0, 0, 1,
                                io, d_prepass_ws, lss_prepass_ws_bytes(N, B), nullptr, side);
        const cudaError_t je = cudaEventRecord(ev_join, side);
        if (ps != LSS_OK || je != cudaSuccess) {
            cudaStreamWaitEvent(stream, ev_join, 0);
            return ps != LSS_OK ? ps : lss_fail(e, LSS_ERR_CUDA, "event record failed");
        }
    }
    cudaError_t ce;
    {
        KernelTimer kt(e, LSS_K_SNOWFALL, stream);
        a.items = d_solve_list;
        {
            unsigned long long *d_ent = (unsigned long long *)(d_sched_hist + 2 * SCHED_BINS);
            unsigned long long *d_sched = d_ent + sched_tiles(N, B);
            const int max_wtiles = (int)((max_n + 31) / 32);
            ce = lss_launch(e, k_sched_key, dim3((unsigned)((max_wtiles + SCHED_KEY_TPB - 1) / SCHED_KEY_TPB), (unsigned)B),
                            SCHED_KEY_TPB, 0, stream, s.d_points, d_off, s.d_cloud_counts, d_order, d_tile_base + B + 1,
                            d_ent, d_sched_hist);
            if (ce == cudaSuccess)
                ce = lss_launch(e, k_sched_sort, (unsigned)((n_wtiles + 256 * SCHED_PER_THREAD - 1) / (256 * SCHED_PER_THREAD)),
                                256, 0, stream, d_ent, d_sched, d_sched_hist, n_wtiles);
            a.sched = d_sched;
            a.n_wtiles = n_wtiles;
        }
        if (ce == cudaSuccess) {
            KernelTimer ks(e, LSS_K_SCAN, stream);
            ce = lss_launch_scan(e, a, stream);
        }
        if (ce == cudaSuccess) {
            KernelTimer ks(e, LSS_K_SOLVE, stream);
            ce = lss_launch_solve(e, a, a.hdr + 1, stream);
        }
    }
    if (ev_join) LSS_CUDA_CHECK(e, cudaStreamWaitEvent(stream, ev_join, 0));
    LSS_CUDA_CHECK(e, ce);
    {
        KernelTimer kt(e, LSS_K_FINALIZE, stream);
        LSS_CUDA_CHECK(e, lss_launch(e, k_keep, dim3(max_tiles, B), KEEP_TPB, 0, stream, a));
    }
    {
        KernelTimer kt(e, LSS_K_SORT, stream);
        LSS_CUDA_CHECK(e, lss_launch(e, k_tile_scan, B, 1024, 0, stream, a.hist_keep, d_tile_base, s.d_out_counts,
                                     s.d_out_stats, a.counters, d_att_cnt, d_att_sum, e->d_sensor));
    }
    {
        KernelTimer kt(e, LSS_K_COMPACT, stream);
        LSS_CUDA_CHECK(e, lss_launch(e, k_scatter, dim3(max_tiles, B), TILE, 0, stream, a.aug, a.code_keep, a.hist_keep, d_off,
                                     s.d_cloud_counts, d_tile_base, s.d_out_points, nullptr, nullptr, nullptr));
    }
    if (want_all) {
        KernelTimer kt(e, LSS_K_COMPACT, stream);
        LSS_CUDA_CHECK(e, lss_launch(e, k_tile_scan, B, 1024, 0, stream, a.hist_all, d_tile_base, nullptr, nullptr, nullptr,
                                     nullptr, nullptr, nullptr));
        LSS_CUDA_CHECK(e, lss_launch(e, k_scatter, dim3(max_tiles, B), TILE, 0, stream, a.aug, a.code_all, a.hist_all, d_off,
                                     s.d_cloud_counts, d_tile_base, s.d_out_full, a.nocc, s.d_out_nocc, s.d_out_perm));
    }
    return LSS_OK;
}
```

### lidar_snow_sim_b200/csrc/solve.cu

```cuda
#include "beam.cuh"

namespace {

constexpr int SOLVE_TPB = 128;
constexpr int SOLVE_WARPS = SOLVE_TPB / 32;
#ifndef LSS_SOLVE_CTAS
#define LSS_SOLVE_CTAS 5
#endif
#ifndef LSS_SOLVE_ARENA
#define LSS_SOLVE_ARENA 160
#endif
constexpr int SOLVE_CTAS_PER_SM = LSS_SOLVE_CTAS;
constexpr int ARENA = LSS_SOLVE_ARENA;
constexpr int SOLVE_LCAP = 128;
static_assert(SOLVE_LCAP + 1 <= ARENA, "a beam with SOLVE_LCAP occluders must fit a round of the arena on its own");
constexpr unsigned FULL = 0xffffffffu;

struct Beam {
    double d, right, left;
    bool straddle;
};

__device__ __forceinline__ void beam_limits(float th32, double half_div, Beam &bm)
{
    const double thd = (double)th32;
    double right = thd - half_div, left = thd + half_div;
    if (right < 0) right += LSS_TWO_PI;
    if (left < 0) left += LSS_TWO_PI;
    if (right > LSS_TWO_PI) right -= LSS_TWO_PI;
    if (left > LSS_TWO_PI) left -= LSS_TWO_PI;
    bm.right = right; bm.left = left; bm.straddle = right > left;
}

__device__ __forceinline__ bool exact_hit(const ParticleRec *rp, const Beam &bm, double &rho, bool &right_hit, bool &left_hit)
{
    rho = rp->rho;
    const double phi = rp->phi, alpha = rp->alpha;
    bool inside = (bm.right <= phi) & (phi <= bm.left);
    if (bm.straddle) inside = inside | ((bm.right - LSS_TWO_PI <= phi) & (phi <= bm.left)) |
                              ((bm.right <= phi) & (phi <= bm.left + LSS_TWO_PI));
    right_hit = within(bm.right - phi, alpha);
    left_hit = within(bm.left - phi, alpha);
    return (rho < bm.d) & (inside | right_hit | left_hit);
}

struct Bucket {
    int e0, e1;
    float th_rel;
    long long pbase;
};

__device__ __forceinline__ Bucket beam_bucket(const DevArgs &a, int plane, float th32)
{
    const double thd = (double)th32;
    const double thm = thd >= LSS_TWO_PI ? thd - LSS_TWO_PI : thd;
    int bk = (int)(thm * a.inv_w);
    bk = bk < 0 ? 0 : (bk >= a.n_buckets ? a.n_buckets - 1 : bk);
    const int32_t *bs = a.bucket_start + (int64_t)plane * (a.n_buckets + 1) + bk;
    Bucket k;
    k.e0 = bs[0];
    k.e1 = bs[1];
    k.th_rel = (float)(thm - (bk + 0.5) * a.w);
    k.pbase = a.plane_off[plane];
    return k;
}

template <class F>
__device__ __forceinline__ int for_each_hit(const DevArgs &a, const Bucket &k, const Beam &bm, float d32, F &&f)
{
    int n = 0;
#pragma unroll 1
    for (int e = k.e0; e < k.e1; e++) {
        const EntryView en = lss_decode(__ldg(&a.entries[e]), a.zbase);
        if (!(en.x < d32)) break;
        if (!(fabsf(en.y - k.th_rel) <= en.z)) continue;
        const long long pi = k.pbase + en.idx;
        double rho;
        bool rh, lh;
        if (exact_hit(a.rec + pi, bm, rho, rh, lh)) { f((int)pi, rho, rh, lh); n++; }
    }
    return n;
}

constexpr int SURV_CAP = 20;

#ifndef LSS_SCAN_CTAS
#define LSS_SCAN_CTAS 10
#endif
__global__ void __launch_bounds__(SNOW_TPB, LSS_SCAN_CTAS) k_scan(DevArgs a)
{
    __shared__ float s_rows[SNOW_WARPS][32 * 5];
    __shared__ int s_idx[SNOW_WARPS][32][SURV_CAP];
    __shared__ unsigned s_hit[SNOW_WARPS][32];
    const int lane = threadIdx.x & 31, wid = threadIdx.x >> 5;
    const int st = blockIdx.x * SNOW_WARPS + wid;
    if (st >= a.n_wtiles) return;
    const unsigned long long se = a.sched[st];
    const int b = (int)((se >> 32) & 0xffffu), w0 = (int)(unsigned)se;
    const int64_t beg = a.cloud_off[b];
    const int n = seg_rows(a.cloud_off, a.cloud_cnt, b);
    const int i = w0 + lane;
    const bool active = i < n;
    const int nf_w = min(32, n - w0) * 5;
    float px = 0, py = 0, pz = 0, pch = 0;
    {
        const float *src = a.pts + (beg + w0) * 5;
#pragma unroll
        for (int q = 0; q < 5; q++) {
            const int f = q * 32 + lane;
            if (f < nf_w) s_rows[wid][f] = __ldcs(src + f);
        }
        __syncwarp();
        if (active) {
            const float *row = &s_rows[wid][5 * lane];
            px = row[0]; py = row[1]; pz = row[2]; pch = row[4];
        }
    }
    const float d32 = __fsqrt_rn(__fadd_rn(__fadd_rn(__fmul_rn(px, px), __fmul_rn(py, py)), __fmul_rn(pz, pz)));
    const int ch = channel_bin(pch);
    float out_l = pch;
    int ns = 0;
    Bucket bkt;
    bkt.e0 = bkt.e1 = 0; bkt.th_rel = 0.0f; bkt.pbase = 0;
    bool slow = false;
    float th32 = 0.0f;
    if (active && ch < LSS_N_CHANNELS) {
        out_l = 0.0f;
        th32 = a.theta ? a.theta[beg + i] : azimuth32(py, px);
        if (th32 < 0.0f) th32 = __fadd_rn(th32, 6.2831855f);
        const int plane = a.order[b * LSS_N_CHANNELS + ch];
        if (plane >= 0 && plane < a.n_planes && th32 == th32) {
            bkt = beam_bucket(a, plane, th32);
            const int e1 = bkt.e1;
            int *pos = s_idx[wid][lane];
            bool stop = false;
#pragma unroll 1
            for (int e = bkt.e0; e < e1 && !stop; e += 4) {
                BroadEntry raw[4];
#pragma unroll
                for (int q = 0; q < 4; q++) raw[q] = __ldg(&a.entries[min(e + q, e1 - 1)]);
#pragma unroll
                for (int q = 0; q < 4; q++) {
                    if (stop || e + q >= e1) continue;
                    const EntryView en = lss_decode(raw[q], a.zbase);
                    if (!(en.x < d32)) { stop = true; continue; }
                    if (!(fabsf(en.y - bkt.th_rel) <= en.z)) continue;
                    if (ns < SURV_CAP) pos[ns] = en.idx;
                    else slow = true;
                    ns++;
                }
            }
        }
    }
    s_hit[wid][lane] = 0u;
    const int mine = slow ? 0 : ns;
    int incl = mine;
#pragma unroll
    for (int sft = 1; sft < 32; sft <<= 1) {
        const int t = __shfl_up_sync(FULL, incl, sft);
        if (lane >= sft) incl += t;
    }
    const int off = incl - mine;
    const int total = __shfl_sync(FULL, incl, 31);
    int hbase = 0;
    if (lane == 0 && total > 0) hbase = atomicAdd(a.hdr + 2, total);
    __syncwarp();
#pragma unroll 1
    for (int s0 = 0; s0 < total; s0 += 32) {
        const int s = s0 + lane;
        int j = 0;
#pragma unroll
        for (int step = 16; step; step >>= 1) {
            const int c = j + step;
            const int oc = __shfl_sync(FULL, off, c & 31);
            if (c < 32 && oc <= s) j = c;
        }
        const int off_j = __shfl_sync(FULL, off, j);
        const int r = s - off_j;
        const long long pbj = __shfl_sync(FULL, bkt.pbase, j);
        Beam bj;
        bj.d = (double)__shfl_sync(FULL, d32, j);
        beam_limits(__shfl_sync(FULL, th32, j), a.half_div, bj);
        bool hit = false;
        double rho = 0.0, a1 = 0.0, a2 = 0.0;
        if (s < total) {
            const long long pi = pbj + s_idx[wid][j][r];
            const ParticleTan tn = a.tan[pi];
            bool rh, lh;
            hit = exact_hit(a.rec + pi, bj, rho, rh, lh);
            a1 = rh ? bj.right : tn.t_right;
            a2 = lh ? bj.left : tn.t_left;
            if (hit) atomicOr(&s_hit[wid][j], 1u << r);
        }
        const int region = __shfl_sync(FULL, hbase, 0) + off_j;
        const bool stored = region + (__shfl_sync(FULL, incl, j) - off_j) <= a.hit_cap;
        __syncwarp();
        if (hit && stored) {
            const int k = region + __popc(s_hit[wid][j] & ((1u << r) - 1u));
            a.hit_a1[k] = a1;
            a.hit_a2[k] = a2;
            a.hit_rho[k] = rho;
        }
    }
    __syncwarp();
    hbase = __shfl_sync(FULL, hbase, 0);
    int L = __popc(s_hit[wid][lane]);
    Beam bm;
    bm.d = (double)d32;
    beam_limits(th32, a.half_div, bm);
    if (slow) L = for_each_hit(a, bkt, bm, d32, [](int, double, bool, bool) {});
    {
        const bool push = L > 0;
        const unsigned pm = __ballot_sync(FULL, push);
        if (push) {
            const int cls = LIST_CLASSES - 1 - min(LIST_CLASSES - 1, 2 * min(L, 63) + (d32 > 40.0f ? 1 : 0));
            const unsigned cm = __match_any_sync(pm, cls);
            const int cl = __ffs(cm) - 1;
            int j = 0;
            if (lane == cl) j = atomicAdd(a.hdr + LIST_CLASSES + cls, __popc(cm));
            j = __shfl_sync(cm, j, cl) + __popc(cm & ((1u << lane) - 1u));
            int *ct = a.chunk_tab + (int64_t)cls * a.chunks_per_class + j / LIST_CHUNK;
            if (j % LIST_CHUNK == 0) atomicExch(ct, atomicAdd(a.hdr, 1) + 1);
            __syncwarp(pm);
            int chunk;
            while ((chunk = *(volatile int *)ct) == 0) {}
            const int hoff = slow ? atomicAdd(a.hdr + 2, L) : hbase + off;
            const bool fits = hoff + (slow ? L : mine) <= a.hit_cap;
            {
                SolveItem it;
                it.key = ((unsigned long long)ch << 56) | ((unsigned long long)cls << 48) |
                         ((unsigned long long)b << 32) | (unsigned)i;
                it.hit_off = fits ? hoff : -1;
                it.L = L;
                it.th32 = th32;
                it.px = s_rows[wid][5 * lane];
                it.py = s_rows[wid][5 * lane + 1];
                it.pz = s_rows[wid][5 * lane + 2];
                a.items[(int64_t)(chunk - 1) * LIST_CHUNK + j % LIST_CHUNK] = it;
            }
            if (fits && slow) {
                int k = hoff;
                for_each_hit(a, bkt, bm, d32, [&](int pi, double rho, bool rh, bool lh) {
                    a.hit_a1[k] = rh ? bm.right : a.tan[pi].t_right;
                    a.hit_a2[k] = lh ? bm.left : a.tan[pi].t_left;
                    a.hit_rho[k] = rho;
                    k++;
                });
            }
        }
    }
    __syncwarp();
    if (active) {
        float *row = &s_rows[wid][5 * lane];
        const float out_i = rintf(row[3]);
        row[3] = out_i;
        row[4] = out_l;
        if (a.nocc) a.nocc[beg + i] = 0;
        a.keep_d[beg + i] = d32;
        a.keep_i[beg + i] = out_i;
        a.keep_tag[beg + i] = (uint8_t)ch;
    }
    __syncwarp();
    {
        float *dst = a.aug + (beg + w0) * 5;
#pragma unroll
        for (int q = 0; q < 5; q++) {
            const int f = q * 32 + lane;
            if (f < nf_w) dst[f] = s_rows[wid][f];
        }
    }
}

__device__ __forceinline__ unsigned long long pack_win(int ks, int ke, int k0)
{
    return (unsigned long long)(unsigned)ks | ((unsigned long long)(unsigned)ke << 11) | ((unsigned long long)(unsigned)k0 << 22);
}

__device__ __forceinline__ void pulse_phase(double r, double &sb, double &cb)
{
    const double ctau = 299792458.0 * 1e-8, inv_ctau = 1.0 / (299792458.0 * 1e-8);
    const double bh = r * inv_ctau;
    const double bl = fma(-bh, ctau, r) * inv_ctau;
    double s, c;
    sincospi(bh, &s, &c);
    const double corr = LSS_PI * bl;
    sb = fma(corr, c, s);
    cb = fma(-corr, s, c);
}

__device__ __forceinline__ void cp_async8(void *dst, const void *src)
{
    asm volatile("cp.async.ca.shared.global [%0], [%1], 8;\n" ::"r"((unsigned)__cvta_generic_to_shared(dst)), "l"(src) : "memory");
}
__device__ __forceinline__ void cp_async_wait_all() { asm volatile("cp.async.wait_all;\n" ::: "memory"); }

#ifdef LSS_SOLVE_PHASE_CLOCKS
enum { PH_FETCH, PH_FILL, PH_CLAIM, PH_PULSES, PH_SWEEP, PH_EVAL, PH_STORE, PH_N };
static_assert(PH_N + 2 + LIST_CLASSES == LSS_DEBUG_SOLVE_PHASE_WORDS, "layout of lss_debug_solve_phases");
__device__ unsigned long long g_solve_phase[LSS_DEBUG_SOLVE_PHASE_WORDS];
#define PHASE_INIT()                                                                                                  \
    __shared__ unsigned long long s_ph[SOLVE_WARPS][PH_N + 1];                                                        \
    if (lane <= PH_N) s_ph[wid][lane] = 0ull;                                                                         \
    unsigned ph_t = (unsigned)clock64();                         \
    unsigned ph_split = 0u
#define PHASE(k)                                                                                                      \
    do {                                                                                                              \
        const unsigned ph_n = (unsigned)clock64();                                                                    \
        if (lane == 0) s_ph[wid][k] += ph_n - ph_t;                                                                   \
        ph_t = ph_n;                                                                                                  \
    } while (0)
#define PHASE_MARK() (ph_split = (unsigned)clock64() - ph_t)
#define PHASE_SPLIT(k0, k1)                                                                                           \
    do {                                                                                                              \
        const unsigned ph_n = (unsigned)clock64();                                                                    \
        const unsigned sp = __reduce_max_sync(FULL, ph_split);                                                        \
        if (lane == 0) { s_ph[wid][k0] += sp; s_ph[wid][k1] += ph_n - ph_t - sp; }                                   \
        ph_t = ph_n;                                                                                                  \
        ph_split = 0u;                                                                                                \
    } while (0)
#define PHASE_TILE(cls, active)                                                                                       \
    do {                                                                                                              \
        const unsigned nb = __popc(__ballot_sync(FULL, active));                                                      \
        if (lane == 0) { s_ph[wid][PH_N]++; atomicAdd(&g_solve_phase[PH_N + 2 + (cls)], (unsigned long long)nb); }    \
    } while (0)
#define PHASE_FLUSH()                                                                                                 \
    do {                                                                                                              \
        if (lane <= PH_N) atomicAdd(&g_solve_phase[lane], s_ph[wid][lane]);                                           \
        if (lane == 0) atomicAdd(&g_solve_phase[PH_N + 1], 1ull);                                                     \
    } while (0)
#else
#define PHASE_INIT()
#define PHASE(k)
#define PHASE_MARK()
#define PHASE_SPLIT(k0, k1)
#define PHASE_TILE(cls, active)
#define PHASE_FLUSH()
#endif

__global__ void __launch_bounds__(SOLVE_TPB, SOLVE_CTAS_PER_SM) k_solve(DevArgs a, int *tile_cursor)
{
    __shared__ double s_arena[SOLVE_WARPS][4][ARENA];
    __shared__ unsigned long long s_piece[SOLVE_WARPS][2 * ARENA];
    __shared__ int s_piece_k[SOLVE_WARPS][2 * ARENA];
    const int lane = threadIdx.x & 31, wid = threadIdx.x >> 5;
    unsigned long long *PD = s_piece[wid];
    int *PK = s_piece_k[wid];
    double *A0 = s_arena[wid][0], *A1 = s_arena[wid][1], *A2 = s_arena[wid][2], *A3 = s_arena[wid][3];
    unsigned long long *W = reinterpret_cast<unsigned long long *>(A2);

    __shared__ int s_tile0[LIST_CLASSES + 1];
    __shared__ int s_cnt[LIST_CLASSES];
    if (wid == 0) {
        int run = 0;
        for (int c0 = 0; c0 < LIST_CLASSES; c0 += 32) {
            const int n = a.hdr[LIST_CLASSES + c0 + lane];
            s_cnt[c0 + lane] = n;
            const int v = (n + 31) >> 5;
            int incl = v;
#pragma unroll
            for (int sft = 1; sft < 32; sft <<= 1) {
                const int t = __shfl_up_sync(FULL, incl, sft);
                if (lane >= sft) incl += t;
            }
            s_tile0[c0 + lane] = run + incl - v;
            run += __shfl_sync(FULL, incl, 31);
        }
        if (lane == 0) s_tile0[LIST_CLASSES] = run;
    }
    __syncthreads();
    const int n_tiles = s_tile0[LIST_CLASSES];
    const double ctau = 299792458.0 * 1e-8;
    const double inv_step = (double)(LSS_M_EXT - 1) / (120 + ctau);
    PHASE_INIT();

    const auto beam_of = [&](int t, int &c, int &j) {
        c = 0;
#pragma unroll
        for (int step = LIST_CLASSES / 2; step; step >>= 1)
            if (s_tile0[c + step] <= t) c += step;
        j = (t - s_tile0[c]) * 32 + lane;
        return t < n_tiles && j < s_cnt[c];
    };
    const auto chunk_of = [&](int c, int j) { return a.chunk_tab[(int64_t)c * a.chunks_per_class + j / LIST_CHUNK]; };
    const auto item_of = [&](int chunk, int j) { return a.items[(int64_t)(chunk - 1) * LIST_CHUNK + j % LIST_CHUNK]; };
    const auto empty_item = [] {
        SolveItem e;
        e.key = 0ull; e.hit_off = 0; e.L = 0; e.th32 = 0.0f; e.px = 0.0f; e.py = 0.0f; e.pz = 0.0f;
        return e;
    };
    int tile = 0;
    if (lane == 0) tile = atomicAdd(tile_cursor, 1);
    tile = __shfl_sync(FULL, tile, 0);
    SolveItem it = empty_item();
    {
        int c, j;
        if (beam_of(tile, c, j)) it = item_of(chunk_of(c, j), j);
    }

    while (tile < n_tiles) {
        int cls, jn;
        const bool active = beam_of(tile, cls, jn);
        int nxt = 0;
        if (lane == 0) nxt = atomicAdd(tile_cursor, 1);
        int nchunk = 0;
        bool fetched = false;
        SolveItem nx = empty_item();
        const auto next_chunk = [&] {
            nxt = __shfl_sync(FULL, nxt, 0);
            if (beam_of(nxt, cls, jn)) nchunk = chunk_of(cls, jn);
        };
        const auto next_item = [&] {
            if (nchunk > 0) nx = item_of(nchunk, jn);
            fetched = true;
        };
        const int b = (int)((it.key >> 32) & 0xffffu);
        const int i = (int)(it.key & 0xffffffffu);
        const int ch = (int)(it.key >> 56);
        const int64_t beg = a.cloud_off[b];
        const float px = it.px, py = it.py, pz = it.pz;
        const float d32 = __fsqrt_rn(__fadd_rn(__fadd_rn(__fmul_rn(px, px), __fmul_rn(py, py)), __fmul_rn(pz, pz)));

        float out_x = px, out_y = py, out_z = pz, out_i = 0.0f, out_l = 0.0f;
        long long att_new_i = -1;
        int n_claim = 0;

        const int L = active ? it.L : 0;
        Beam bm;
        bm.d = (double)d32;
        beam_limits(it.th32, a.half_div, bm);

        if (L > SOLVE_LCAP) raise_status(a.status, LSS_ERR_OCCLUDER_OVERFLOW);
        const int need = (L > 0 && L <= SOLVE_LCAP) ? L + 1 : 0;
        PHASE_TILE(cls, active);
        PHASE(PH_FETCH);

        unsigned remaining = __ballot_sync(FULL, need > 0);
        while (remaining) {
            const bool rem = (remaining >> lane) & 1u;
            const int mine = rem ? need : 0;
            int incl = mine;
#pragma unroll
            for (int s = 1; s < 32; s <<= 1) {
                const int t = __shfl_up_sync(FULL, incl, s);
                if (lane >= s) incl += t;
            }
            const bool in_round = rem && incl <= ARENA;
            remaining &= ~__ballot_sync(FULL, in_round);
            const int off = incl - mine;
            const int total = (int)__reduce_max_sync(FULL, in_round ? (unsigned)incl : 0u);
            int n_pulses = 0;
            double amax = 0.0;
            double best = 0.0;
            int kbest = 0;

#pragma unroll 1
            for (int s0 = 0; s0 < total; s0 += 32) {
                const int s = s0 + lane;
                int j = 0;
#pragma unroll
                for (int step = 16; step; step >>= 1) {
                    const int c = j + step;
                    const int oc = __shfl_sync(FULL, off, c & 31);
                    if (c < 32 && oc <= s) j = c;
                }
                const int r = s - __shfl_sync(FULL, off, j);
                const int Lj = __shfl_sync(FULL, L, j);
                const int hoj = __shfl_sync(FULL, it.hit_off, j);
                const int inr = __shfl_sync(FULL, (int)in_round, j);
                if (s < total && inr && r < Lj && hoj >= 0) {
                    cp_async8(&A0[s], &a.hit_a1[hoj + r]);
                    cp_async8(&A1[s], &a.hit_a2[hoj + r]);
                    cp_async8(&A2[s], &a.hit_rho[hoj + r]);
                }
            }
            cp_async_wait_all();
            __syncwarp();
            if (in_round && it.hit_off < 0) {
                const Bucket bkt = beam_bucket(a, a.order[b * LSS_N_CHANNELS + ch], it.th32);
                int s = off;
                for_each_hit(a, bkt, bm, d32, [&](int pi, double rho, bool rh, bool lh) {
                    A0[s] = rh ? bm.right : a.tan[pi].t_right;
                    A1[s] = lh ? bm.left : a.tan[pi].t_left;
                    A2[s] = rho;
                    s++;
                });
            }
            __syncwarp();
            if (!fetched) next_chunk();
            PHASE(PH_FILL);

            if (in_round) {
#pragma unroll 1
                for (int p = 1; p < L; p++) {
                    const double rho = A2[off + p];
                    if (!(A2[off + p - 1] > rho)) continue;
                    const double a1 = A0[off + p], a2 = A1[off + p];
                    int q = p - 1;
#pragma unroll 1
                    while (q >= 0 && A2[off + q] > rho) { A0[off + q + 1] = A0[off + q]; A1[off + q + 1] = A1[off + q]; A2[off + q + 1] = A2[off + q]; q--; }
                    A0[off + q + 1] = a1; A1[off + q + 1] = a2; A2[off + q + 1] = rho;
                }

                double rb = bm.right;
                if (bm.straddle) rb = bm.right - LSS_TWO_PI;
                int nu = 0, P = 0;
                double ep_min = fmin(rb, bm.left), ep_max = fmax(rb, bm.left), claimed_total = 0.0;
#pragma unroll 1
                for (int j = 0; j < L; j++) {
                    double lo = A0[off + j];
                    const double hi = A1[off + j], rho = A2[off + j];
                    if (bm.straddle && lo > hi) lo -= LSS_TWO_PI;
                    ep_min = fmin(ep_min, fmin(lo, hi));
                    ep_max = fmax(ep_max, fmax(lo, hi));
                    if (!(lo < hi)) continue;
                    bool contained = false;
                    double cov = 0.0, nlo = lo, nhi = hi;
                    int w = 0;
#pragma unroll 1
                    for (int u = 0; u < nu; u++) {
                        const double ul = A0[off + u], uh = A1[off + u];
                        if ((ul <= lo) && (hi <= uh)) { contained = true; break; }
                        if (ul <= hi && uh >= lo) {
                            const double ov = fmin(hi, uh) - fmax(lo, ul);
                            if (ov > 0.0) cov += ov;
                            nlo = fmin(nlo, ul);
                            nhi = fmax(nhi, uh);
                        } else {
                            A0[off + w] = ul; A1[off + w] = uh; w++;
                        }
                    }
                    if (contained) continue;
                    const double claimed = (hi - lo) - cov;
                    claimed_total += claimed;
                    A0[off + w] = nlo; A1[off + w] = nhi;
                    nu = w + 1;
                    double ratio = claimed / a.div_rad;
                    ratio = ratio < 0 ? 0 : (ratio > 1 ? 1 : ratio);
                    A2[off + P] = rho;
                    A3[off + P] = ratio;
                    P++;
                }
                n_claim = P;
                double ratio_hard = ((ep_max - ep_min) - claimed_total) / a.div_rad;
                ratio_hard = ratio_hard < 0 ? 0 : (ratio_hard > 1 ? 1 : ratio_hard);
                PHASE_MARK();

                if (P > 0) {
                    const double beta_0 = 1 * 1e-06 / LSS_PI;
                    const double i_orig = 0.9 * a.sensor->max_intensity[ch];
                    const double A = (i_orig / beta_0) * beta_0;
                    bool bad = false;
#pragma unroll 1
                    for (int j = 0; j < P; j++) {
                        const double r = A2[off + j], ratio = A3[off + j];
                        const int ks = (int)ceil(r * 10);
                        const int ke = (int)(floor((r + ctau) * 10) + 1);
                        bad |= (ke > LSS_M_EXT) || (ks < 0);
                        double sb, cb;
                        pulse_phase(r, sb, cb);
                        const double amp = (A * ratio * xsi64(r)) / (r * r);
                        amax = fmax(amax, amp);
                        A0[off + j] = amp;
                        A1[off + j] = sb;
                        A3[off + j] = cb;
                        W[off + j] = pack_win(ks, ke, (int)rint((r + ctau / 2) * inv_step));
                    }
                    {
                        const int ks = (int)ceilf(__fmul_rn(d32, 10.0f));
                        const int ke = (int)(floorf(__fmul_rn(__fadd_rn(d32, (float)ctau), 10.0f)) + 1.0f);
                        bad |= (ke > LSS_M_EXT) || (ks < 0);
                        double sb, cb;
                        pulse_phase(bm.d, sb, cb);
                        const double amp = (A * ratio_hard * xsi32(d32)) / (double)__fmul_rn(d32, d32);
                        amax = fmax(amax, amp);
                        A0[off + P] = amp;
                        A1[off + P] = sb;
                        A3[off + P] = cb;
                        W[off + P] = pack_win(ks, ke, (int)rint((bm.d + ctau / 2) * inv_step));
                    }
                    if (bad) raise_status(a.status, LSS_ERR_RANGE_INDEX);
                    else n_pulses = P + 1;
                }
            }
            PHASE_SPLIT(PH_CLAIM, PH_PULSES);
            if (!fetched) next_item();

            int np_mine = 0;
            if (n_pulses > 0) {
                const double lb = 0.99 * amax;
                double asum = 0.0;
                int qa = 0, qb = -1, nxt = 0;
                int ks_n = (int)(W[off] & 2047u);
                int ke_a = 0;
                int k = ks_n;
                unsigned long long *pd = PD + 2 * off;
#pragma unroll 1
                for (;;) {
#pragma unroll 1
                    while (ks_n <= k) {
                        qb = nxt++;
                        asum += A0[off + qb];
                        ks_n = nxt < n_pulses ? (int)(W[off + nxt] & 2047u) : 4096;
                    }
#pragma unroll 1
                    while (qa <= qb) {
                        ke_a = (int)((W[off + qa] >> 11) & 2047u);
                        if (ke_a > k) break;
                        asum -= A0[off + qa];
                        qa++;
                    }
                    if (qa > qb) {
                        asum = 0.0;
                        if (nxt >= n_pulses) break;
                        k = ks_n;
                        continue;
                    }
                    const int pend = min(ke_a, ks_n);
                    if (asum * 1.0001 >= lb)
                        pd[np_mine++] = (unsigned long long)(unsigned)k | ((unsigned long long)(unsigned)pend << 11) |
                                        ((unsigned long long)(unsigned)(off + qa) << 22) | ((unsigned long long)(unsigned)(off + qb) << 32);
                    k = pend;
                }
            }
            int pincl = np_mine;
#pragma unroll
            for (int sft = 1; sft < 32; sft <<= 1) {
                const int t = __shfl_up_sync(FULL, pincl, sft);
                if (lane >= sft) pincl += t;
            }
            const int pex = pincl - np_mine;
            const int ptotal = __shfl_sync(FULL, pincl, 31);
            __syncwarp();
            PHASE(PH_SWEEP);
            {
                const float step = (float)((120 + ctau) / (double)(LSS_M_EXT - 1));
                const float ctau_f = (float)ctau;
#pragma unroll 1
                for (int f0 = 0; f0 < ptotal; f0 += 32) {
                    const int f = f0 + lane;
                    int j = 0;
#pragma unroll
                    for (int stp = 16; stp; stp >>= 1) {
                        const int c = j + stp;
                        const int oc = __shfl_sync(FULL, pex, c & 31);
                        if (c < 32 && oc <= f) j = c;
                    }
                    const int slot = 2 * __shfl_sync(FULL, off, j) + (f - __shfl_sync(FULL, pex, j));
                    if (f < ptotal) {
                        const unsigned long long d = PD[slot];
                        const int lo = (int)(d & 2047u), hi = (int)((d >> 11) & 2047u);
                        const int qa = (int)((d >> 22) & 1023u), qb = (int)((d >> 32) & 1023u);
                        double pbest = 0.0;
                        int pk = lo;
                        auto eval = [&](int c) {
                            const double2 t = __ldg(&a.wtab[c]);
                            double v = 0.0;
#pragma unroll 1
                            for (int q = qa; q <= qb; q++) {
                                const double sn = t.x * A3[q] - t.y * A1[q];
                                v += A0[q] * (sn * sn);
                            }
                            if (v > pbest) { pbest = v; pk = c; }
                        };
                        int kc;
                        bool all = false;
                        if (qa == qb) {
                            kc = (int)((W[qa] >> 22) & 2047u);
                        } else {
                            float zx = 0.0f, zy = 0.0f, asum = 0.0f;
#pragma unroll 1
                            for (int q = qa; q <= qb; q++) {
                                const float A = (float)A0[q], sn = (float)A1[q], cs = (float)A3[q];
                                zx += A * (cs * cs - sn * sn);
                                zy += A * (2.0f * sn * cs);
                                asum += A;
                            }
                            all = zx * zx + zy * zy < 1e-6f * asum * asum;
                            const float r0 = (atan2f(zy, zx) + 3.14159265f) * (ctau_f * 0.15915494f);
                            const float rc = 0.5f * (float)(lo + hi - 1) * step;
                            kc = (int)rintf((r0 + rintf((rc - r0) / ctau_f) * ctau_f) / step);
                        }
                        const int c_lo = all ? lo : max(lo, min(hi - 1, kc - 1));
                        const int c_hi = all ? hi - 1 : min(hi - 1, max(lo, kc + 1));
#pragma unroll 1
                        for (int c = c_lo; c <= c_hi; c++) eval(c);
                        PD[slot] = (unsigned long long)__double_as_longlong(pbest);
                        PK[slot] = pk;
                    }
                }
            }
            __syncwarp();
#pragma unroll 1
            for (int r = 0; r < np_mine; r++) {
                const double v = __longlong_as_double((long long)PD[2 * off + r]);
                if (v > best) { best = v; kbest = PK[2 * off + r]; }
            }
            __syncwarp();
            PHASE(PH_EVAL);

            if (n_pulses > 0) {
                const double max_i = a.sensor->max_intensity[ch];
                const double min_i = a.sensor->min_intensity[ch];
                const double d_max = ((double)kbest / 10) - (ctau / 2);
                const double q1 = 1 - d_max / 120;
                double i_max = best + max_i * a.sensor->focal_slope[ch] * fabs(a.sensor->focal_offset[ch] - q1 * q1);
                i_max = i_max < min_i ? min_i : (i_max > max_i ? max_i : i_max);
                const long long new_i = (long long)i_max;
                if (fabs(d_max - bm.d) < 2 * (1.0 / 10)) {
                    out_l = 1.0f;
                    att_new_i = new_i;
                } else {
                    out_l = 2.0f;
                    const double sc = d_max / bm.d;
                    out_x = (float)((double)px * sc);
                    out_y = (float)((double)py * sc);
                    out_z = (float)((double)pz * sc);
                }
                if (new_i < 0) raise_status(a.status, LSS_ERR_NEGATIVE_INTENSITY);
                double ci = (double)new_i;
                ci = ci < min_i ? min_i : (ci > max_i ? max_i : ci);
                out_i = (float)ci;
            }
            __syncwarp();
            PHASE(PH_STORE);
        }
        if (!fetched) { next_chunk(); next_item(); }

        if (active) {
            if (out_l != 0.0f) {
                const float ri = rintf(out_i);
                float *row = a.aug + (beg + i) * 5;
                row[0] = out_x; row[1] = out_y; row[2] = out_z; row[3] = ri; row[4] = out_l;
                a.keep_i[beg + i] = ri;
                a.keep_tag[beg + i] = keep_tag_of(ch, out_l);
            }
            if (a.nocc) a.nocc[beg + i] = n_claim;
        }
        {
            const bool on = att_new_i >= 0;
            const int key = b * LSS_N_CHANNELS + (ch < LSS_N_CHANNELS ? ch : 0);
            const unsigned mk = __match_any_sync(FULL, on ? key : -1);
            if (on && lane == __ffs(mk) - 1) atomicAdd(a.att_cnt + key, (unsigned)__popc(mk));
            const unsigned mb = __match_any_sync(FULL, on ? b : -1);
            const unsigned sum = __reduce_add_sync(mb, on ? (unsigned)att_new_i : 0u);
            if (on && lane == __ffs(mb) - 1) atomicAdd(&a.att_sum[b], (unsigned long long)sum);
        }
        PHASE(PH_STORE);
        tile = nxt;
        it = nx;
    }
    PHASE_FLUSH();
}

}

namespace {
__global__ void k_debug_azimuth(const float *y, const float *x, float *out, int64_t n)
{
    const int64_t i = (int64_t)blockIdx.x * blockDim.x + threadIdx.x;
    if (i < n) out[i] = azimuth32(y[i], x[i]);
}
}

extern "C" lss_status lss_debug_azimuth(lss_engine *e, const float *d_y, const float *d_x, int64_t n, float *d_out, void *stream)
{
    if (!e || !d_y || !d_x || !d_out || n < 0) return LSS_ERR_INVALID_ARG;
    if (n == 0) return LSS_OK;
    DeviceGuard g(e->device);
    LSS_CUDA_CHECK(e, lss_launch(e, k_debug_azimuth, (unsigned)((n + 255) / 256), 256, 0, (cudaStream_t)stream, d_y, d_x,
                                 d_out, n));
    return LSS_OK;
}

extern "C" lss_status lss_debug_solve_phases(lss_engine *e, int reset, uint64_t *h_out, int n)
{
    if (!e || (h_out && n < LSS_DEBUG_SOLVE_PHASE_WORDS)) return LSS_ERR_INVALID_ARG;
#ifdef LSS_SOLVE_PHASE_CLOCKS
    DeviceGuard g(e->device);
    LSS_CUDA_CHECK(e, cudaDeviceSynchronize());
    if (h_out) LSS_CUDA_CHECK(e, cudaMemcpyFromSymbol(h_out, g_solve_phase, sizeof(g_solve_phase)));
    if (reset) {
        static const unsigned long long zero[LSS_DEBUG_SOLVE_PHASE_WORDS] = {};
        LSS_CUDA_CHECK(e, cudaMemcpyToSymbol(g_solve_phase, zero, sizeof(zero)));
    }
    return LSS_OK;
#else
    (void)reset;
    return lss_fail(e, LSS_ERR_INVALID_ARG, "lss_debug_solve_phases: the library was built without -DLSS_SOLVE_PHASE_CLOCKS");
#endif
}

cudaError_t lss_launch_scan(lss_engine *e, const DevArgs &a, cudaStream_t stream)
{
    return lss_launch(e, k_scan, (unsigned)((a.n_wtiles + SNOW_WARPS - 1) / SNOW_WARPS), SNOW_TPB, 0, stream, a);
}

cudaError_t lss_launch_solve(lss_engine *e, const DevArgs &a, int *tile_cursor, cudaStream_t stream)
{
    return lss_launch(e, k_solve, (unsigned)(e->n_sm * SOLVE_CTAS_PER_SM), SOLVE_TPB, 0, stream, a, tile_cursor);
}
```

### lidar_snow_sim_b200/csrc/wet_ground.cu

```cuda
#include <climits>
#include <vector>

#include "segments.cuh"

namespace {

constexpr int WET_TPB = 256;
constexpr int WET_TILE = 1024;

struct WetArgs {
    const float *pts;
    const int64_t *cloud_off;
    const int32_t *cloud_cnt;
    const CloudPre *cp;
    double delta, noise_floor, power_factor;
    const double *f_wet;
    int flat_earth, replace;
    uint8_t *cls;
    double *new_i;
    float *out;
    double *out_i64;
    int32_t *out_counts;
    int32_t *out_passthrough;
    SegTiles seg;
};

__device__ __forceinline__ int wet_passthrough(const CloudPre &cp)
{
    if (cp.n_ground < 1000) return 1;
    return lss_intensity_range_ok(cp.ymax) ? 0 : 2;
}

struct Fresnel { double rs, ts, rp, tp, aout; };

__device__ __forceinline__ Fresnel fresnel_power(double ain, double nair, double nw)
{
    Fresnel f;
    double a = sin(ain) * nair / nw;
    a = a < -1 ? -1 : (a > 1 ? 1 : a);
    const double aout = asin(a);
    const double ci = cos(ain), co = cos(aout);
    const double pft = ci * nair / nw / co;
    double rs = (nair * ci - nw * co) / (nair * ci + nw * co);
    double ts = 2 * nair * ci / (nair * ci + nw * co);
    double rp = (nw * ci - nair * co) / (nw * ci + nair * co);
    double tp = 2 * nair * ci / (nw * ci + nair * co);
    f.rs = rs * rs;
    f.ts = ts * ts / pft;
    f.rp = rp * rp;
    f.tp = tp * tp / pft;
    f.aout = aout;
    return f;
}

__global__ void __launch_bounds__(WET_TPB) k_wet_points(WetArgs a)
{
    const int b = blockIdx.y;
    const CloudPre cp = a.cp[b];
    const int64_t beg = a.cloud_off[b];
    const int n = seg_rows(a.cloud_off, a.cloud_cnt, b);
    const bool pass = wet_passthrough(cp) != 0;
    const double f_wet = a.f_wet[b];
    for (int i = blockIdx.x * WET_TPB + threadIdx.x; i < n; i += gridDim.x * WET_TPB) {
        const float *r = a.pts + (beg + i) * 5;
        const double x = r[0], y = r[1], z = r[2], inten = r[3];
        const double pw = lss_plane_dot(x, y, z, cp.w);
        const double hgt = pw + cp.h;
        const bool ground = !pass && (hgt < a.delta) && (hgt > -a.delta);
        uint8_t c = 0;
        if (ground) {
            const double d = sqrt((x * x + y * y) + z * z);
            const double ang = a.flat_earth ? acos(-(z) / (d * 1.0)) : acos(pw / (d * cp.nw));
            const double ca = cos(ang);
            const double rel_out = a.power_factor * (cp.lin[0] * d + cp.lin[1]);
            const double noise = a.noise_floor * (cp.pmin[0] * d + cp.pmin[1]);
            const double refl = inten / ca / rel_out;
            const double rho = refl < 0.05 ? 0.05 : (refl > 1 ? 1 : refl);
            const Fresnel f1 = fresnel_power(ang, 1.0003, 1.33);
            const Fresnel f2 = fresnel_power(f1.aout, 1.33, 1.0003);
            const double ts = f1.ts * rho * f2.ts / (1 - rho * f2.rs);
            const double tp = f1.tp * rho * f2.tp / (1 - rho * f2.rp);
            const double t = fmax(tp, ts);
            const double tw = (1 - f_wet) * refl + f_wet * t / ang;
            double ni = rel_out * ca * tw;
            ni = ni < 0 ? 0 : (ni > inten ? inten : ni);
            const double thr = noise * ca;
            if (ni < thr) ni = 0;
            c = (ni > thr) ? 1 : 2;
            a.new_i[beg + i] = ni;
        }
        a.cls[beg + i] = c;
    }
}

__global__ void __launch_bounds__(WET_TILE) k_wet_scatter(WetArgs a)
{
    const int b = blockIdx.y, tile = blockIdx.x;
    const CloudPre &cp = a.cp[b];
    const int pass_code = wet_passthrough(cp);
    const bool pass = pass_code != 0;
    if (tile == 0 && threadIdx.x == 0) {
        a.out_counts[b] = a.seg.total[0][b] + a.seg.total[1][b];
        if (a.out_passthrough) a.out_passthrough[b] = pass_code;
    }
    const int n = seg_rows(a.cloud_off, a.cloud_cnt, b);
    if (tile * WET_TILE >= n) return;
    const int64_t beg = a.cloud_off[b];
    const int n_non = pass ? n : n - cp.n_ground;
    const int i = tile * WET_TILE + threadIdx.x;
    const int c = i < n ? a.cls[beg + i] : 2;
    const int r = seg_rank<2, WET_TILE>(c < 2 ? c : -1, a.seg, b, tile);
    if (r >= 0) {
        const float *s = a.pts + (beg + i) * 5;
        const int dst = (c == 0) ? r : n_non + r;
        float *o = a.out + (beg + dst) * 5;
        o[0] = s[0]; o[1] = s[1]; o[2] = s[2];
        const double inten = (c == 1) ? a.new_i[beg + i] : (double)s[3];
        o[3] = (float)inten;
        o[4] = pass ? s[4] : ((c == 1) ? 1.0f : (a.replace ? 0.0f : s[4]));
        if (a.out_i64) a.out_i64[beg + dst] = inten;
    }
}

void *wet_carve(WsCarve &c, WetArgs &a, int64_t n_total, int n_clouds)
{
    a.cloud_off = c.take<int64_t>(n_clouds + 1);
    a.f_wet = c.take<double>(n_clouds);
    a.cls = c.take<uint8_t>(n_total);
    a.new_i = c.take<double>(n_total);
    a.seg = seg_take(c, n_total, n_clouds, WET_TILE, 2);
    a.seg.total[0] = c.take<int32_t>((int64_t)n_clouds * 2);
    return c.take<char>(lss_prepass_ws_bytes(n_total, n_clouds));
}

lss_status wet_ground_run(lss_engine *e, const float *d_points, const int64_t *h_cloud_offsets,
                          const int32_t *d_cloud_counts, int n_clouds, const double *h_water_height,
                          double pavement_depth, double noise_floor, double power_factor, int flat_earth, double delta,
                          int replace, const double *h_plane_in, const int32_t *h_ymins_in, float *d_out_points,
                          double *d_out_intensity64, int32_t *d_out_counts, int32_t *d_out_passthrough,
                          double *d_out_plane, double *d_out_fit, int32_t *d_out_ymins, void *d_workspace,
                          int64_t workspace_bytes, void *stream, bool latch_range)
{
    if (!e) return LSS_ERR_INVALID_ARG;
    BatchGeometry g;
    if (lss_status rc = lss_batch_geometry(e, h_cloud_offsets, n_clouds, WET_TILE, g)) return rc;
    if (!d_out_points || !d_out_counts || !d_workspace) return lss_fail(e, LSS_ERR_INVALID_ARG, "null argument");
    const int B = n_clouds;
    const int64_t N = g.n;
    DeviceGuard dg(e->device);
    cudaStream_t st = (cudaStream_t)stream;
    if (B == 0 || N == 0) {
        ZeroRegions z;
        z.add(d_out_counts, sizeof(int32_t) * B);
        LSS_CUDA_CHECK(e, lss_zero_async(e, z, st));
        return LSS_OK;
    }
    if (!d_points) return lss_fail(e, LSS_ERR_INVALID_ARG, "null points");
    WetArgs a;
    WsCarve c{(char *)d_workspace};
    void *d_prepass_ws = wet_carve(c, a, N, B);
    if (workspace_bytes < c.used) return lss_fail(e, LSS_ERR_WORKSPACE, "workspace too small");
    if (lss_status rc = lss_prepass_check(e, h_cloud_offsets, B, h_plane_in != nullptr)) return rc;
    a.seg.total[1] = a.seg.total[0] + B;
    int64_t *d_off = (int64_t *)a.cloud_off;
    LSS_CUDA_CHECK(e, lss_stage_geometry(e, h_cloud_offsets, B, g.tile_base, d_off, (int32_t *)a.seg.tile_base, st));
    void *cp_ptr = nullptr;
    PrepassIO io;
    io.h_plane_in = h_plane_in;
    io.h_ymins_in = h_ymins_in;
    io.d_plane_out = d_out_plane;
    io.d_fit_out = d_out_fit;
    io.d_ymins_out = d_out_ymins;
    io.range_min_ground = latch_range ? 1000 : INT_MAX;
    if (lss_status rc = lss_prepass_run(e, d_points, d_off, d_cloud_counts, h_cloud_offsets, B, delta, noise_floor,
                                        flat_earth, 1, 0, io, d_prepass_ws, lss_prepass_ws_bytes(N, B), &cp_ptr, st))
        return rc;
    a.pts = d_points;
    a.cloud_cnt = d_cloud_counts;
    a.cp = (const CloudPre *)cp_ptr;
    a.delta = delta;
    a.noise_floor = noise_floor;
    a.power_factor = power_factor;
    {
        std::vector<double> f_wet(B);
        for (int b = 0; b < B; b++) {
            const double f = h_water_height[b] / pavement_depth;
            f_wet[b] = f < 0 ? 0 : (f > 1 ? 1 : f);
        }
        LSS_CUDA_CHECK(e, lss_stage_upload(e, (double *)a.f_wet, f_wet.data(), sizeof(double) * B, st));
    }
    a.flat_earth = flat_earth;
    a.replace = replace;
    a.out = d_out_points;
    a.out_i64 = d_out_intensity64;
    a.out_counts = d_out_counts;
    a.out_passthrough = d_out_passthrough;
    const int max_tiles = (int)std::max<int64_t>(1, (g.max_n + WET_TILE - 1) / WET_TILE);
    const int nblk = (int)std::max<int64_t>(1, std::min<int64_t>(1024, (g.max_n + WET_TPB * 4 - 1) / (WET_TPB * 4)));
    {
        KernelTimer kt(e, LSS_K_WET, st);
        LSS_CUDA_CHECK(e, lss_launch(e, k_wet_points, dim3(nblk, B), WET_TPB, 0, st, a));
    }
    KernelTimer kt(e, LSS_K_COMPACT, st);
    LSS_CUDA_CHECK(e, lss_launch(e, k_seg_count_codes<2, WET_TILE>, dim3(max_tiles, B), WET_TILE, 0, st, a.cls, a.cloud_off,
                                 a.cloud_cnt, a.seg));
    LSS_CUDA_CHECK(e, lss_launch(e, k_seg_scan<2>, B, SEG_SCAN_TPB, 0, st, a.seg));
    LSS_CUDA_CHECK(e, lss_launch(e, k_wet_scatter, dim3(max_tiles, B), WET_TILE, 0, st, a));
    return LSS_OK;
}

}

extern "C" {

int64_t lss_wet_ground_workspace_bytes(int64_t n_total, int n_clouds)
{
    if (n_total < 0 || n_clouds < 0) return -1;
    WsCarve c;
    WetArgs a;
    wet_carve(c, a, n_total, n_clouds);
    return c.used;
}

lss_status lss_wet_ground_batch(lss_engine *e, const float *d_points, const int64_t *h_cloud_offsets,
                                const int32_t *d_cloud_counts, int n_clouds, double water_height, double pavement_depth,
                                double noise_floor, double power_factor, int flat_earth, double delta, int replace,
                                const double *h_plane_in, const int32_t *h_ymins_in, float *d_out_points,
                                double *d_out_intensity64, int32_t *d_out_counts, int32_t *d_out_passthrough,
                                double *d_out_plane, double *d_out_fit, int32_t *d_out_ymins, void *d_workspace,
                                int64_t workspace_bytes, void *stream)
{
    const std::vector<double> heights((size_t)std::max(n_clouds, 0), water_height);
    return wet_ground_run(e, d_points, h_cloud_offsets, d_cloud_counts, n_clouds, heights.data(), pavement_depth,
                          noise_floor, power_factor, flat_earth, delta, replace, h_plane_in, h_ymins_in, d_out_points,
                          d_out_intensity64, d_out_counts, d_out_passthrough, d_out_plane, d_out_fit, d_out_ymins,
                          d_workspace, workspace_bytes, stream, true);
}

lss_status lss_wet_ground_batch_params(lss_engine *e, const float *d_points, const int64_t *h_cloud_offsets,
                                       const int32_t *d_cloud_counts, int n_clouds, const double *h_water_height,
                                       double pavement_depth, double noise_floor, double power_factor, int flat_earth,
                                       double delta, int replace, const double *h_plane_in, const int32_t *h_ymins_in,
                                       float *d_out_points, double *d_out_intensity64, int32_t *d_out_counts,
                                       int32_t *d_out_passthrough, double *d_out_plane, double *d_out_fit,
                                       int32_t *d_out_ymins, void *d_workspace, int64_t workspace_bytes, void *stream)
{
    if (!e) return LSS_ERR_INVALID_ARG;
    if (!h_water_height && n_clouds > 0) return lss_fail(e, LSS_ERR_INVALID_ARG, "null water heights");
    return wet_ground_run(e, d_points, h_cloud_offsets, d_cloud_counts, n_clouds, h_water_height, pavement_depth,
                          noise_floor, power_factor, flat_earth, delta, replace, h_plane_in, h_ymins_in, d_out_points,
                          d_out_intensity64, d_out_counts, d_out_passthrough, d_out_plane, d_out_fit, d_out_ymins,
                          d_workspace, workspace_bytes, stream, false);
}

}
```

Baseline: 4.753 billion.

## Batch staging uploads and zeroing into one kernel and launch dependents with PDL

Merges the separate host-to-device staging copies and zero-fill launches into a single combined stage-copy kernel, driven by one pinned buffer and one event per call. Also launches most downstream kernels with programmatic dependent launch (griddepcontrol trigger/wait), so each kernel's launch latency overlaps the tail of its predecessor. The goal is to cut per-call launch count and inter-kernel gaps in a pipeline dominated by many small kernels. It adds complexity around event lifetimes (the StageDone destructor records an event) and depends on every kernel calling wait before it reads upstream results.

```diff
diff --git a/lidar_snow_sim_b200/csrc/api.cu b/lidar_snow_sim_b200/csrc/api.cu
--- a/lidar_snow_sim_b200/csrc/api.cu
+++ b/lidar_snow_sim_b200/csrc/api.cu
@@ -323,7 +323,6 @@
     int64_t pre_bytes;
     int64_t *d_off = poly_carve(c, d_pre, pre_bytes, geo.n, n_clouds);
     if (workspace_bytes < c.used) return lss_fail(e, LSS_ERR_WORKSPACE, "workspace too small");
-    LSS_CUDA_CHECK(e, lss_stage_upload(e, d_off, h_cloud_offsets, sizeof(int64_t) * (n_clouds + 1), st));
     PrepassIO io;
     io.h_plane_in = h_plane_in;
     io.h_ymins_in = h_ymins_in;
@@ -331,6 +330,12 @@
     io.d_plane_out = d_plane_out;
     io.d_fit_out = d_fit_out;
     io.d_ymins_out = d_ymins_out;
+    io.staged = true;
+    StageDone stage_done;
+    StageList l;
+    l.upload(d_off, h_cloud_offsets, sizeof(int64_t) * (n_clouds + 1));
+    lss_prepass_stage(l, io, d_pre, geo.n, n_clouds);
+    LSS_CUDA_CHECK(e, lss_stage(e, l, st, &stage_done));
     return lss_prepass_run(e, d_points, d_off, nullptr, h_cloud_offsets, n_clouds, 0.5, noise_floor, 0, 0, 1, io,
                            d_pre, pre_bytes, nullptr, st);
 }
diff --git a/lidar_snow_sim_b200/csrc/common.cuh b/lidar_snow_sim_b200/csrc/common.cuh
--- a/lidar_snow_sim_b200/csrc/common.cuh
+++ b/lidar_snow_sim_b200/csrc/common.cuh
@@ -140,6 +140,28 @@
     return cudaGetLastError();
 }
 
+__device__ __forceinline__ void lss_pdl_wait() { asm volatile("griddepcontrol.wait;\n" ::: "memory"); }
+__device__ __forceinline__ void lss_pdl_trigger() { asm volatile("griddepcontrol.launch_dependents;\n" ::: "memory"); }
+
+template <typename... P, typename... A>
+[[nodiscard]] inline cudaError_t lss_launch_pdl(lss_engine *e, void (*kernel)(P...), dim3 grid, dim3 block, size_t smem,
+                                                cudaStream_t stream, A &&...args)
+{
+    cudaLaunchAttribute attr[1];
+    attr[0].id = cudaLaunchAttributeProgrammaticStreamSerialization;
+    attr[0].val.programmaticStreamSerializationAllowed = 1;
+    cudaLaunchConfig_t cfg = {};
+    cfg.gridDim = grid;
+    cfg.blockDim = block;
+    cfg.dynamicSmemBytes = smem;
+    cfg.stream = stream;
+    cfg.attrs = attr;
+    cfg.numAttrs = 1;
+    const cudaError_t err = cudaLaunchKernelEx(&cfg, kernel, std::forward<A>(args)...);
+    e->launches++;
+    return err;
+}
+
 inline cudaError_t lss_side_stream(lss_engine *e, cudaStream_t *stream, cudaEvent_t *ev_fork, cudaEvent_t *ev_join)
 {
     cudaError_t err;
@@ -157,61 +179,114 @@
     return cudaSuccess;
 }
 
-static __global__ void k_stage_copy(uint32_t *dst, const uint32_t *src, int n_words)
-{
-    for (int i = blockIdx.x * blockDim.x + threadIdx.x; i < n_words; i += gridDim.x * blockDim.x) dst[i] = src[i];
-}
-
-inline cudaError_t lss_stage_upload(lss_engine *e, void *dst, const void *src, size_t bytes, cudaStream_t stream)
-{
-    if (bytes == 0) return cudaSuccess;
-    if (bytes % 4 != 0 || ((uintptr_t)dst & 3) != 0) return cudaErrorInvalidValue;
-    lss_engine::StageSlot &sl = e->stage[e->stage_next];
-    e->stage_next = (e->stage_next + 1) % lss_engine::N_STAGE;
-    cudaError_t err;
-    if (!sl.done) {
-        if ((err = cudaEventCreateWithFlags(&sl.done, cudaEventDisableTiming)) != cudaSuccess) return err;
-    } else if ((err = cudaEventSynchronize(sl.done)) != cudaSuccess) {
-        return err;
-    }
-    if (sl.cap < bytes) {
-        if (sl.host) cudaFreeHost(sl.host);
-        sl.host = nullptr; sl.cap = 0;
-        const size_t cap = bytes < 4096 ? 4096 : bytes * 2;
-        if ((err = cudaHostAlloc(&sl.host, cap, cudaHostAllocMapped)) != cudaSuccess) return err;
-        sl.cap = cap;
-    }
-    memcpy(sl.host, src, bytes);
-    const int n_words = (int)(bytes / 4);
-    const int blocks = n_words >= 1 << 16 ? 64 : (n_words + 1023) / 1024;
-    if ((err = lss_launch(e, k_stage_copy, blocks, 256, 0, stream, (uint32_t *)dst, (const uint32_t *)sl.host, n_words)) !=
-        cudaSuccess)
-        return err;
-    return cudaEventRecord(sl.done, stream);
-}
-
 struct ZeroRegions {
-    static constexpr int MAX = 6;
+    static constexpr int MAX = 8;
     uint32_t *p[MAX];
     unsigned long long words[MAX];
     int n = 0;
     void add(void *ptr, size_t bytes) { if (ptr && bytes) { p[n] = (uint32_t *)ptr; words[n] = (bytes + 3) / 4; n++; } }
 };
-static __global__ void k_zero_regions(ZeroRegions r)
-{
-    uint32_t *p = r.p[blockIdx.y];
-    const unsigned long long n = r.words[blockIdx.y];
+
+struct StageList {
+    static constexpr int MAX = 8;
+    uint32_t *dst[MAX];
+    const uint32_t *src[MAX];
+    unsigned long long words[MAX];
+    int n = 0;
+    bool bad = false;
+    ZeroRegions zero;
+    void upload(void *d, const void *h, size_t bytes)
+    {
+        if (bytes == 0) return;
+        if (n == MAX || bytes % 4 != 0 || ((uintptr_t)d & 3) != 0) { bad = true; return; }
+        dst[n] = (uint32_t *)d; src[n] = (const uint32_t *)h; words[n] = bytes / 4; n++;
+    }
+};
+static __global__ void k_stage_copy(StageList s)
+{
+    lss_pdl_trigger();
+    const int r = blockIdx.y;
     const unsigned long long stride = (unsigned long long)gridDim.x * blockDim.x;
-    for (unsigned long long i = (unsigned long long)blockIdx.x * blockDim.x + threadIdx.x; i < n; i += stride) p[i] = 0u;
-}
-inline cudaError_t lss_zero_async(lss_engine *e, const ZeroRegions &r, cudaStream_t stream)
-{
-    if (r.n == 0) return cudaSuccess;
+    const unsigned long long i0 = (unsigned long long)blockIdx.x * blockDim.x + threadIdx.x;
+    if (r < s.n) {
+        uint32_t *dst = s.dst[r];
+        const uint32_t *src = s.src[r];
+        for (unsigned long long i = i0; i < s.words[r]; i += stride) dst[i] = src[i];
+    } else {
+        uint32_t *p = s.zero.p[r - s.n];
+        for (unsigned long long i = i0; i < s.zero.words[r - s.n]; i += stride) p[i] = 0u;
+    }
+}
+
+struct StageDone {
+    cudaEvent_t ev = nullptr;
+    cudaStream_t stream = nullptr;
+    StageDone() = default;
+    StageDone(const StageDone &) = delete;
+    StageDone &operator=(const StageDone &) = delete;
+    ~StageDone() { if (ev) cudaEventRecord(ev, stream); }
+};
+
+inline cudaError_t lss_stage(lss_engine *e, StageList l, cudaStream_t stream, StageDone *done = nullptr)
+{
+    if (l.bad) return cudaErrorInvalidValue;
+    if (l.n + l.zero.n == 0) return cudaSuccess;
+    size_t bytes = 0;
     unsigned long long mx = 0;
-    for (int i = 0; i < r.n; i++) mx = r.words[i] > mx ? r.words[i] : mx;
+    for (int k = 0; k < l.n; k++) {
+        bytes += (size_t)align_up((int64_t)l.words[k] * 4, 16);
+        mx = l.words[k] > mx ? l.words[k] : mx;
+    }
+    for (int k = 0; k < l.zero.n; k++) mx = l.zero.words[k] > mx ? l.zero.words[k] : mx;
+    cudaError_t err;
+    lss_engine::StageSlot *sl = nullptr;
+    if (bytes) {
+        sl = &e->stage[e->stage_next];
+        e->stage_next = (e->stage_next + 1) % lss_engine::N_STAGE;
+        if (!sl->done) {
+            if ((err = cudaEventCreateWithFlags(&sl->done, cudaEventDisableTiming)) != cudaSuccess) return err;
+        } else if ((err = cudaEventSynchronize(sl->done)) != cudaSuccess) {
+            return err;
+        }
+        if (sl->cap < bytes) {
+            if (sl->host) cudaFreeHost(sl->host);
+            sl->host = nullptr; sl->cap = 0;
+            const size_t cap = bytes < 4096 ? 4096 : bytes * 2;
+            if ((err = cudaHostAlloc(&sl->host, cap, cudaHostAllocMapped)) != cudaSuccess) return err;
+            sl->cap = cap;
+        }
+        size_t off = 0;
+        for (int k = 0; k < l.n; k++) {
+            char *h = (char *)sl->host + off;
+            memcpy(h, l.src[k], l.words[k] * 4);
+            l.src[k] = (const uint32_t *)h;
+            off += (size_t)align_up((int64_t)l.words[k] * 4, 16);
+        }
+    }
     const unsigned long long cap = 4ull * e->n_sm;
     const unsigned blocks = (unsigned)((mx + 1023) / 1024 < cap ? (mx + 1023) / 1024 : cap);
-    return lss_launch(e, k_zero_regions, dim3(blocks ? blocks : 1, r.n), 256, 0, stream, r);
+    if ((err = lss_launch(e, k_stage_copy, dim3(blocks ? blocks : 1, l.n + l.zero.n), 256, 0, stream, l)) != cudaSuccess)
+        return err;
+    if (!sl) return cudaSuccess;
+    if (!done) return cudaEventRecord(sl->done, stream);
+    if (done->ev && (err = cudaEventRecord(done->ev, done->stream)) != cudaSuccess) return err;
+    done->ev = sl->done;
+    done->stream = stream;
+    return cudaSuccess;
+}
+
+inline cudaError_t lss_stage_upload(lss_engine *e, void *dst, const void *src, size_t bytes, cudaStream_t stream)
+{
+    StageList l;
+    l.upload(dst, src, bytes);
+    return lss_stage(e, l, stream);
+}
+
+inline cudaError_t lss_zero_async(lss_engine *e, const ZeroRegions &r, cudaStream_t stream)
+{
+    StageList l;
+    l.zero = r;
+    return lss_stage(e, l, stream);
 }
 
 enum { LSS_K_SORT = 0, LSS_K_PREPASS = 1, LSS_K_SNOWFALL = 2, LSS_K_COMPACT = 3, LSS_K_FINALIZE = 4, LSS_K_WET = 5,
@@ -341,7 +416,9 @@
     double *d_fit_out = nullptr;
     int32_t *d_ymins_out = nullptr;
     int range_min_ground = 3;
-};
+    bool staged = false;
+};
+void lss_prepass_stage(StageList &l, const PrepassIO &io, void *d_ws, int64_t n_total, int n_clouds);
 lss_status lss_prepass_run(lss_engine *e, const float *d_pts, const int64_t *d_cloud_off, const int32_t *d_cloud_cnt,
                            const int64_t *h_cloud_off, int n_clouds, double delta, double noise_floor, int flat_earth,
                            int range64, int raise_few_ground, const PrepassIO &io, void *d_ws, int64_t ws_bytes,
diff --git a/lidar_snow_sim_b200/csrc/prepass.cu b/lidar_snow_sim_b200/csrc/prepass.cu
--- a/lidar_snow_sim_b200/csrc/prepass.cu
+++ b/lidar_snow_sim_b200/csrc/prepass.cu
@@ -663,6 +663,18 @@
     return c.used;
 }
 
+void lss_prepass_stage(StageList &l, const PrepassIO &io, void *d_ws, int64_t n_total, int n_clouds)
+{
+    WsCarve c{(char *)d_ws};
+    PreArgs a;
+    double *d_plane;
+    int32_t *d_ymins_in;
+    prepass_carve(c, a, d_plane, d_ymins_in, n_total, n_clouds);
+    l.zero.add(a.cp, (size_t)((char *)a.rec_cnt - (char *)a.cp) + sizeof(int) * n_clouds);
+    if (io.h_ymins_in) l.upload(d_ymins_in, io.h_ymins_in, sizeof(int32_t) * HIST_NX * n_clouds);
+    if (io.h_plane_in) l.upload(d_plane, io.h_plane_in, sizeof(double) * 4 * n_clouds);
+}
+
 static size_t gather_dyn_smem(int64_t max_n) { return sizeof(int) * ((size_t)(max_n + 31) / 32 + 2); }
 
 static int64_t largest_cloud(const int64_t *h_cloud_off, int n_clouds)
@@ -726,24 +738,18 @@
     a.flat_earth = flat_earth;
     a.have_plane = h_plane_in != nullptr;
     a.status = e->d_status;
-    a.ymins_in = nullptr;
-    if (io.h_ymins_in) {
-        LSS_CUDA_CHECK(e, lss_stage_upload(e, d_ymins_in, io.h_ymins_in, sizeof(int32_t) * HIST_NX * B, stream));
-        a.ymins_in = d_ymins_in;
-    }
+    a.ymins_in = io.h_ymins_in ? d_ymins_in : nullptr;
     if (cloudpre_out) *cloudpre_out = a.cp;
     const int64_t max_n = largest_cloud(h_cloud_off, B);
     int nblk = (int)std::min<int64_t>(a.max_blocks, std::max<int64_t>(1, (max_n + PP_TPB * 8 - 1) / (PP_TPB * 8)));
-
-    {
-        ZeroRegions z;
-        z.add(a.cp, (size_t)((char *)a.rec_cnt - (char *)a.cp) + sizeof(int) * B);
-        LSS_CUDA_CHECK(e, lss_zero_async(e, z, stream));
+    if (!io.staged) {
+        StageList l;
+        lss_prepass_stage(l, io, d_ws, N, B);
+        LSS_CUDA_CHECK(e, lss_stage(e, l, stream));
     }
     {
         KernelTimer kt(e, LSS_K_PREPASS, stream);
         if (h_plane_in) {
-            LSS_CUDA_CHECK(e, lss_stage_upload(e, d_plane, h_plane_in, sizeof(double) * 4 * B, stream));
             LSS_CUDA_CHECK(e, lss_launch(e, k_set_plane, (B + 127) / 128, 128, 0, stream, a, d_plane));
         } else {
             const int max_tiles = (int)std::max<int64_t>(1, (max_n + WTILE - 1) / WTILE);
diff --git a/lidar_snow_sim_b200/csrc/segments.cuh b/lidar_snow_sim_b200/csrc/segments.cuh
--- a/lidar_snow_sim_b200/csrc/segments.cuh
+++ b/lidar_snow_sim_b200/csrc/segments.cuh
@@ -67,6 +67,8 @@
 __global__ void __launch_bounds__(TILE) k_seg_count_codes(const uint8_t *code, const int64_t *cloud_off,
                                                           const int32_t *cloud_cnt, SegTiles s)
 {
+    lss_pdl_trigger();
+    lss_pdl_wait();
     const int b = blockIdx.y, tile = blockIdx.x;
     if (tile >= s.tile_base[b + 1] - s.tile_base[b]) return;
     const int i = tile * TILE + threadIdx.x;
@@ -81,6 +83,8 @@
 template <int K>
 __global__ void __launch_bounds__(SEG_SCAN_TPB) k_seg_scan(SegTiles s)
 {
+    lss_pdl_trigger();
+    lss_pdl_wait();
     __shared__ __align__(16) int warp_sum[K][SEG_SCAN_TPB / 32];
     __shared__ int run[K];
     const int b = blockIdx.x;
diff --git a/lidar_snow_sim_b200/csrc/snowfall.cu b/lidar_snow_sim_b200/csrc/snowfall.cu
--- a/lidar_snow_sim_b200/csrc/snowfall.cu
+++ b/lidar_snow_sim_b200/csrc/snowfall.cu
@@ -9,6 +9,8 @@
                                                             const int32_t *__restrict__ order, const int32_t *__restrict__ wtile_base,
                                                             unsigned long long *ent, int *hist)
 {
+    lss_pdl_trigger();
+    lss_pdl_wait();
     const int b = blockIdx.y, t = blockIdx.x * SCHED_KEY_TPB + threadIdx.x;
     const int64_t beg = cloud_off[b];
     const int n_slot = (int)(cloud_off[b + 1] - beg);
@@ -30,6 +32,8 @@
 __global__ void __launch_bounds__(256) k_sched_sort(const unsigned long long *__restrict__ in, unsigned long long *out,
                                                     int *hist, int n)
 {
+    lss_pdl_trigger();
+    lss_pdl_wait();
     __shared__ int base[SCHED_BINS], cnt[SCHED_BINS], blk[SCHED_BINS];
     const int first = blockIdx.x * (256 * SCHED_PER_THREAD);
     for (int c = threadIdx.x; c < SCHED_BINS; c += 256) cnt[c] = 0;
@@ -80,6 +84,8 @@
 
 __global__ void __launch_bounds__(KEEP_TPB) k_keep(DevArgs a)
 {
+    lss_pdl_trigger();
+    lss_pdl_wait();
     __shared__ unsigned h_keep[NBINS], h_all[NBINS];
     __shared__ int s_cnt[2];
     const int b = blockIdx.y, tile = blockIdx.x;
@@ -160,6 +166,8 @@
                                                      const unsigned *att_cnt, const unsigned long long *att_sum,
                                                      const SensorConst *sensor)
 {
+    lss_pdl_trigger();
+    lss_pdl_wait();
     __shared__ unsigned bin_total[NBINS];
     __shared__ double att_term[LSS_N_CHANNELS];
     const int b = blockIdx.x;
@@ -232,6 +240,8 @@
                                                    float *__restrict__ out, const int32_t *__restrict__ nocc_in,
                                                    int32_t *__restrict__ nocc_out, int32_t *__restrict__ perm_out)
 {
+    lss_pdl_trigger();
+    lss_pdl_wait();
     __shared__ unsigned warp_cnt[TILE / 32][NBINS];
     const int b = blockIdx.y, tile = blockIdx.x;
     const int64_t beg = cloud_off[b];
@@ -353,25 +363,30 @@
     unsigned *d_att_cnt = (unsigned *)((char *)a.counters + att_cnt_off(B));
     unsigned long long *d_att_sum = (unsigned long long *)((char *)d_att_cnt + (int64_t)B * LSS_N_CHANNELS * 4);
 
+    StageDone stage_done;
+    StageList l;
     g.tile_base.insert(g.tile_base.end(), wg.tile_base.begin(), wg.tile_base.end());
-    LSS_CUDA_CHECK(e, lss_stage_geometry(e, s.h_cloud_offsets, B, g.tile_base, d_off, d_tile_base, stream));
-    LSS_CUDA_CHECK(e, lss_stage_upload(e, d_order, s.h_order, sizeof(int32_t) * B * LSS_N_CHANNELS, stream));
-    if (s.h_thresh_poly)
-        LSS_CUDA_CHECK(e, lss_stage_upload(e, d_thresh, s.h_thresh_poly, sizeof(double) * 3 * B, stream));
-    {
-        ZeroRegions z;
-        z.add(a.counters, counters_bytes(B));
-        z.add(s.d_out_stats, sizeof(double) * 4 * B);
-        if (N == 0 || B == 0) {
-            z.add(s.d_out_counts, sizeof(int32_t) * B);
-            LSS_CUDA_CHECK(e, lss_zero_async(e, z, stream));
-            return LSS_OK;
-        }
-        z.add(a.hdr, LIST_HDR_BYTES);
-        z.add(a.chunk_tab, (size_t)LIST_CLASSES * a.chunks_per_class * 4);
-        z.add(d_sched_hist, (size_t)SCHED_BINS * 2 * 4);
-        LSS_CUDA_CHECK(e, lss_zero_async(e, z, stream));
-    }
+    l.upload(d_off, s.h_cloud_offsets, sizeof(int64_t) * (B + 1));
+    l.upload(d_tile_base, g.tile_base.data(), sizeof(int32_t) * g.tile_base.size());
+    l.upload(d_order, s.h_order, sizeof(int32_t) * B * LSS_N_CHANNELS);
+    if (s.h_thresh_poly) l.upload(d_thresh, s.h_thresh_poly, sizeof(double) * 3 * B);
+    l.zero.add(a.counters, counters_bytes(B));
+    l.zero.add(s.d_out_stats, sizeof(double) * 4 * B);
+    if (N == 0 || B == 0) {
+        l.zero.add(s.d_out_counts, sizeof(int32_t) * B);
+        LSS_CUDA_CHECK(e, lss_stage(e, l, stream, &stage_done));
+        return LSS_OK;
+    }
+    l.zero.add(a.hdr, LIST_HDR_BYTES);
+    l.zero.add(a.chunk_tab, (size_t)LIST_CLASSES * a.chunks_per_class * 4);
+    l.zero.add(d_sched_hist, (size_t)SCHED_BINS * 2 * 4);
+    PrepassIO io;
+    io.h_plane_in = s.h_plane_in;
+    io.h_ymins_in = s.h_ymins_in;
+    io.d_poly_out = d_thresh;
+    io.staged = true;
+    if (device_prepass) lss_prepass_stage(l, io, d_prepass_ws, N, B);
+    LSS_CUDA_CHECK(e, lss_stage(e, l, stream, &stage_done));
 
     a.rec = s.ts->d_rec;
     a.tan = s.ts->d_tan;
@@ -408,10 +423,6 @@
         LSS_CUDA_CHECK(e, lss_side_stream(e, &side, &ev_fork, &ev_join));
         LSS_CUDA_CHECK(e, cudaEventRecord(ev_fork, stream));
         LSS_CUDA_CHECK(e, cudaStreamWaitEvent(side, ev_fork, 0));
-        PrepassIO io;
-        io.h_plane_in = s.h_plane_in;
-        io.h_ymins_in = s.h_ymins_in;
-        io.d_poly_out = d_thresh;
         lss_status ps = lss_prepass_run(e, s.d_points, d_off, s.d_cloud_counts, s.h_cloud_offsets, B, 0.5, s.noise_floor, 0, 0, 1,
                                 io, d_prepass_ws, lss_prepass_ws_bytes(N, B), nullptr, side);
         const cudaError_t je = cudaEventRecord(ev_join, side);
@@ -428,12 +439,12 @@
             unsigned long long *d_ent = (unsigned long long *)(d_sched_hist + 2 * SCHED_BINS);
             unsigned long long *d_sched = d_ent + sched_tiles(N, B);
             const int max_wtiles = (int)((max_n + 31) / 32);
-            ce = lss_launch(e, k_sched_key, dim3((unsigned)((max_wtiles + SCHED_KEY_TPB - 1) / SCHED_KEY_TPB), (unsigned)B),
-                            SCHED_KEY_TPB, 0, stream, s.d_points, d_off, s.d_cloud_counts, d_order, d_tile_base + B + 1,
-                            d_ent, d_sched_hist);
+            ce = lss_launch_pdl(e, k_sched_key, dim3((unsigned)((max_wtiles + SCHED_KEY_TPB - 1) / SCHED_KEY_TPB), (unsigned)B),
+                                SCHED_KEY_TPB, 0, stream, s.d_points, d_off, s.d_cloud_counts, d_order, d_tile_base + B + 1,
+                                d_ent, d_sched_hist);
             if (ce == cudaSuccess)
-                ce = lss_launch(e, k_sched_sort, (unsigned)((n_wtiles + 256 * SCHED_PER_THREAD - 1) / (256 * SCHED_PER_THREAD)),
-                                256, 0, stream, d_ent, d_sched, d_sched_hist, n_wtiles);
+                ce = lss_launch_pdl(e, k_sched_sort, (unsigned)((n_wtiles + 256 * SCHED_PER_THREAD - 1) / (256 * SCHED_PER_THREAD)),
+                                    256, 0, stream, d_ent, d_sched, d_sched_hist, n_wtiles);
             a.sched = d_sched;
             a.n_wtiles = n_wtiles;
         }
@@ -450,24 +461,24 @@
     LSS_CUDA_CHECK(e, ce);
     {
         KernelTimer kt(e, LSS_K_FINALIZE, stream);
-        LSS_CUDA_CHECK(e, lss_launch(e, k_keep, dim3(max_tiles, B), KEEP_TPB, 0, stream, a));
+        LSS_CUDA_CHECK(e, lss_launch_pdl(e, k_keep, dim3(max_tiles, B), KEEP_TPB, 0, stream, a));
     }
     {
         KernelTimer kt(e, LSS_K_SORT, stream);
-        LSS_CUDA_CHECK(e, lss_launch(e, k_tile_scan, B, 1024, 0, stream, a.hist_keep, d_tile_base, s.d_out_counts,
-                                     s.d_out_stats, a.counters, d_att_cnt, d_att_sum, e->d_sensor));
+        LSS_CUDA_CHECK(e, lss_launch_pdl(e, k_tile_scan, B, 1024, 0, stream, a.hist_keep, d_tile_base, s.d_out_counts,
+                                         s.d_out_stats, a.counters, d_att_cnt, d_att_sum, e->d_sensor));
     }
     {
         KernelTimer kt(e, LSS_K_COMPACT, stream);
-        LSS_CUDA_CHECK(e, lss_launch(e, k_scatter, dim3(max_tiles, B), TILE, 0, stream, a.aug, a.code_keep, a.hist_keep, d_off,
-                                     s.d_cloud_counts, d_tile_base, s.d_out_points, nullptr, nullptr, nullptr));
+        LSS_CUDA_CHECK(e, lss_launch_pdl(e, k_scatter, dim3(max_tiles, B), TILE, 0, stream, a.aug, a.code_keep, a.hist_keep, d_off,
+                                         s.d_cloud_counts, d_tile_base, s.d_out_points, nullptr, nullptr, nullptr));
     }
     if (want_all) {
         KernelTimer kt(e, LSS_K_COMPACT, stream);
-        LSS_CUDA_CHECK(e, lss_launch(e, k_tile_scan, B, 1024, 0, stream, a.hist_all, d_tile_base, nullptr, nullptr, nullptr,
-                                     nullptr, nullptr, nullptr));
-        LSS_CUDA_CHECK(e, lss_launch(e, k_scatter, dim3(max_tiles, B), TILE, 0, stream, a.aug, a.code_all, a.hist_all, d_off,
-                                     s.d_cloud_counts, d_tile_base, s.d_out_full, a.nocc, s.d_out_nocc, s.d_out_perm));
+        LSS_CUDA_CHECK(e, lss_launch_pdl(e, k_tile_scan, B, 1024, 0, stream, a.hist_all, d_tile_base, nullptr, nullptr, nullptr,
+                                         nullptr, nullptr, nullptr));
+        LSS_CUDA_CHECK(e, lss_launch_pdl(e, k_scatter, dim3(max_tiles, B), TILE, 0, stream, a.aug, a.code_all, a.hist_all, d_off,
+                                         s.d_cloud_counts, d_tile_base, s.d_out_full, a.nocc, s.d_out_nocc, s.d_out_perm));
     }
     return LSS_OK;
 }
diff --git a/lidar_snow_sim_b200/csrc/solve.cu b/lidar_snow_sim_b200/csrc/solve.cu
--- a/lidar_snow_sim_b200/csrc/solve.cu
+++ b/lidar_snow_sim_b200/csrc/solve.cu
@@ -93,7 +93,9 @@
     __shared__ int s_idx[SNOW_WARPS][32][SURV_CAP];
     __shared__ unsigned s_hit[SNOW_WARPS][32];
     const int lane = threadIdx.x & 31, wid = threadIdx.x >> 5;
+    lss_pdl_trigger();
     const int st = blockIdx.x * SNOW_WARPS + wid;
+    lss_pdl_wait();
     if (st >= a.n_wtiles) return;
     const unsigned long long se = a.sched[st];
     const int b = (int)((se >> 32) & 0xffffu), w0 = (int)(unsigned)se;
@@ -350,6 +352,8 @@
 
     __shared__ int s_tile0[LIST_CLASSES + 1];
     __shared__ int s_cnt[LIST_CLASSES];
+    lss_pdl_trigger();
+    lss_pdl_wait();
     if (wid == 0) {
         int run = 0;
         for (int c0 = 0; c0 < LIST_CLASSES; c0 += 32) {
@@ -790,12 +794,17 @@
 #endif
 }
 
+#ifndef LSS_PDL_SOLVE
+#define LSS_PDL_SOLVE 1
+#endif
 cudaError_t lss_launch_scan(lss_engine *e, const DevArgs &a, cudaStream_t stream)
 {
-    return lss_launch(e, k_scan, (unsigned)((a.n_wtiles + SNOW_WARPS - 1) / SNOW_WARPS), SNOW_TPB, 0, stream, a);
+    return lss_launch_pdl(e, k_scan, (unsigned)((a.n_wtiles + SNOW_WARPS - 1) / SNOW_WARPS), SNOW_TPB, 0, stream, a);
 }
 
 cudaError_t lss_launch_solve(lss_engine *e, const DevArgs &a, int *tile_cursor, cudaStream_t stream)
 {
-    return lss_launch(e, k_solve, (unsigned)(e->n_sm * SOLVE_CTAS_PER_SM), SOLVE_TPB, 0, stream, a, tile_cursor);
-}
+    const unsigned grid = (unsigned)(e->n_sm * SOLVE_CTAS_PER_SM);
+    if (LSS_PDL_SOLVE) return lss_launch_pdl(e, k_solve, grid, SOLVE_TPB, 0, stream, a, tile_cursor);
+    return lss_launch(e, k_solve, grid, SOLVE_TPB, 0, stream, a, tile_cursor);
+}
diff --git a/lidar_snow_sim_b200/csrc/wet_ground.cu b/lidar_snow_sim_b200/csrc/wet_ground.cu
--- a/lidar_snow_sim_b200/csrc/wet_ground.cu
+++ b/lidar_snow_sim_b200/csrc/wet_ground.cu
@@ -55,6 +55,8 @@
 
 __global__ void __launch_bounds__(WET_TPB) k_wet_points(WetArgs a)
 {
+    lss_pdl_trigger();
+    lss_pdl_wait();
     const int b = blockIdx.y;
     const CloudPre cp = a.cp[b];
     const int64_t beg = a.cloud_off[b];
@@ -95,6 +97,8 @@
 
 __global__ void __launch_bounds__(WET_TILE) k_wet_scatter(WetArgs a)
 {
+    lss_pdl_trigger();
+    lss_pdl_wait();
     const int b = blockIdx.y, tile = blockIdx.x;
     const CloudPre &cp = a.cp[b];
     const int pass_code = wet_passthrough(cp);
@@ -163,8 +167,6 @@
     if (lss_status rc = lss_prepass_check(e, h_cloud_offsets, B, h_plane_in != nullptr)) return rc;
     a.seg.total[1] = a.seg.total[0] + B;
     int64_t *d_off = (int64_t *)a.cloud_off;
-    LSS_CUDA_CHECK(e, lss_stage_geometry(e, h_cloud_offsets, B, g.tile_base, d_off, (int32_t *)a.seg.tile_base, st));
-    void *cp_ptr = nullptr;
     PrepassIO io;
     io.h_plane_in = h_plane_in;
     io.h_ymins_in = h_ymins_in;
@@ -172,6 +174,22 @@
     io.d_fit_out = d_out_fit;
     io.d_ymins_out = d_out_ymins;
     io.range_min_ground = latch_range ? 1000 : INT_MAX;
+    io.staged = true;
+    StageDone stage_done;
+    {
+        std::vector<double> f_wet(B);
+        for (int b = 0; b < B; b++) {
+            const double f = h_water_height[b] / pavement_depth;
+            f_wet[b] = f < 0 ? 0 : (f > 1 ? 1 : f);
+        }
+        StageList l;
+        l.upload(d_off, h_cloud_offsets, sizeof(int64_t) * (B + 1));
+        l.upload((int32_t *)a.seg.tile_base, g.tile_base.data(), sizeof(int32_t) * g.tile_base.size());
+        l.upload((double *)a.f_wet, f_wet.data(), sizeof(double) * B);
+        lss_prepass_stage(l, io, d_prepass_ws, N, B);
+        LSS_CUDA_CHECK(e, lss_stage(e, l, st, &stage_done));
+    }
+    void *cp_ptr = nullptr;
     if (lss_status rc = lss_prepass_run(e, d_points, d_off, d_cloud_counts, h_cloud_offsets, B, delta, noise_floor,
                                         flat_earth, 1, 0, io, d_prepass_ws, lss_prepass_ws_bytes(N, B), &cp_ptr, st))
         return rc;
@@ -181,14 +199,6 @@
     a.delta = delta;
     a.noise_floor = noise_floor;
     a.power_factor = power_factor;
-    {
-        std::vector<double> f_wet(B);
-        for (int b = 0; b < B; b++) {
-            const double f = h_water_height[b] / pavement_depth;
-            f_wet[b] = f < 0 ? 0 : (f > 1 ? 1 : f);
-        }
-        LSS_CUDA_CHECK(e, lss_stage_upload(e, (double *)a.f_wet, f_wet.data(), sizeof(double) * B, st));
-    }
     a.flat_earth = flat_earth;
     a.replace = replace;
     a.out = d_out_points;
@@ -199,13 +209,13 @@
     const int nblk = (int)std::max<int64_t>(1, std::min<int64_t>(1024, (g.max_n + WET_TPB * 4 - 1) / (WET_TPB * 4)));
     {
         KernelTimer kt(e, LSS_K_WET, st);
-        LSS_CUDA_CHECK(e, lss_launch(e, k_wet_points, dim3(nblk, B), WET_TPB, 0, st, a));
+        LSS_CUDA_CHECK(e, lss_launch_pdl(e, k_wet_points, dim3(nblk, B), WET_TPB, 0, st, a));
     }
     KernelTimer kt(e, LSS_K_COMPACT, st);
-    LSS_CUDA_CHECK(e, lss_launch(e, k_seg_count_codes<2, WET_TILE>, dim3(max_tiles, B), WET_TILE, 0, st, a.cls, a.cloud_off,
-                                 a.cloud_cnt, a.seg));
-    LSS_CUDA_CHECK(e, lss_launch(e, k_seg_scan<2>, B, SEG_SCAN_TPB, 0, st, a.seg));
-    LSS_CUDA_CHECK(e, lss_launch(e, k_wet_scatter, dim3(max_tiles, B), WET_TILE, 0, st, a));
+    LSS_CUDA_CHECK(e, lss_launch_pdl(e, k_seg_count_codes<2, WET_TILE>, dim3(max_tiles, B), WET_TILE, 0, st, a.cls,
+                                     a.cloud_off, a.cloud_cnt, a.seg));
+    LSS_CUDA_CHECK(e, lss_launch_pdl(e, k_seg_scan<2>, B, SEG_SCAN_TPB, 0, st, a.seg));
+    LSS_CUDA_CHECK(e, lss_launch_pdl(e, k_wet_scatter, dim3(max_tiles, B), WET_TILE, 0, st, a));
     return LSS_OK;
 }
 
```

After: 5.081 billion (median of 6 runs). +6.9%, better.
